# IVRL/NoiseDiff

Measured on AMD Instinct MI355X. Metric: sampled RAW patches/sec (256x256x4, 1000-step DDPM), higher is better.
Workload: dtype f32; 1 GPU; NoiseDiffNet dim=64, 256x256x4 patches, 1000-step DDPM (sigmoid2, pred_v), 16 patches per GPU; a step = one reverse-diffusion step (U-Net forward + fused posterior/noise update) over the per-GPU batch; patches/s = n_gpus*16/(1000*s_per_step); global_batch=16, launch=hipGraph replay, noise=device Philox4x32-10

## Files before the change

include/noisediff_hip.h:

```cpp
#ifndef NOISEDIFF_HIP_H
#define NOISEDIFF_HIP_H

#include <stdint.h>

#ifdef __cplusplus
extern "C" {
#endif

#define ND_E_BADARG   (-1)
#define ND_E_SHAPE    (-2)
#define ND_E_ALIGN    (-3)
#define ND_E_STATE    (-4)

int         nd_version(void);
const char* nd_last_error(void);
int         nd_device_arch(char* buf, int n);


enum nd_prologue {
    ND_PRO_NONE        = 0,
    ND_PRO_AFFINE_SILU = 1,
    ND_PRO_AFFINE_MAP_SILU = 2,
    ND_PRO_LAYERNORM   = 3,
    ND_PRO_SILU        = 4,
    ND_PRO_LEAKY       = 5,
    ND_PRO_LEAKY_SECOND = 6,
    ND_PRO_AFFINE_GENMAP_SILU = 7
};

typedef struct nd_src {
    const float* p0;
    const float* p1;
    int32_t c0, c1;
    int32_t ld0, ld1;
    int32_t mode;
    int32_t upsample;
    int32_t unshuffle;
    int32_t map_blocked;
    const float* mad;
    const float* map;
    const float* vec;
    const float* gamma;
    const float* beta;
    const float* rowstats;
} nd_src;

enum nd_act { ND_ACT_NONE = 0, ND_ACT_GELU = 1, ND_ACT_SILU = 2 };


typedef struct nd_conv3x3 {
    nd_src   src;
    const float* weight;
    const float* bias;
    float*   out;
    float*   stats;
    float*   slot_count;
    int32_t  B, H, W;
    int32_t  cin, cout, ldo;
} nd_conv3x3;

int nd_conv3x3_nhwc_f32(const nd_conv3x3* d, void* stream);
enum nd_conv3x3_kernel { ND_CONV3X3_DIRECT = 0, ND_CONV3X3_WINO = 1, ND_CONV3X3_WINO2 = 2, ND_CONV3X3_WINO4 = 3, ND_CONV3X3_WINO4_16 = 4 };
int nd_conv3x3_takes(int kernel, const nd_conv3x3* d, int splits);
int nd_conv3x3_stat_slots(int H, int W, int cout, int B);
int nd_conv3x3_tiling_id(int B, int H, int W, int cout);
int64_t nd_pack_conv3x3_weight_floats(int cin, int cout);
int nd_pack_conv3x3_weight(const float* oihw, float* packed, int cin, int cout, void* stream);
int nd_pack_conv3x3_weight_dgrad(const float* oihw_fwd, float* packed, int cin, int cout, void* stream);

int nd_conv3x3_wino_nhwc_f32(const nd_conv3x3* d, void* stream);
int nd_conv3x3_wino2_nhwc_f32(const nd_conv3x3* d, void* stream);
int nd_conv3x3_wino_stat_slots(int H, int W);
int64_t nd_pack_conv3x3_wino_weight_floats(int cin, int cout);
int nd_pack_conv3x3_wino_weight(const float* oihw, float* packed, int cin, int cout, void* stream);
int nd_pack_conv3x3_wino_weight_dgrad(const float* oihw_fwd, float* packed, int cin, int cout, void* stream);

int nd_conv3x3_wino4_nhwc_f32(const nd_conv3x3* d, void* stream);
int nd_conv3x3_wino4_16_nhwc_f32(const nd_conv3x3* d, void* stream);
int nd_conv3x3_wino4_stat_slots(int H, int W);
int64_t nd_pack_conv3x3_wino4_weight_floats(int cin, int cout);
int nd_pack_conv3x3_wino4_weight(const float* oihw, float* packed, int cin, int cout, void* stream);
int nd_pack_conv3x3_wino4_weight_dgrad(const float* oihw_fwd, float* packed, int cin, int cout, void* stream);
typedef struct nd_pack_item {
    const float* w;
    float*       packed;
    int32_t      cin, cout, transposed, reserved;
} nd_pack_item;
int nd_pack_conv3x3_wino4_weights_batch(const nd_pack_item* items_dev, int n_items, void* stream);
int nd_conv3x3_wino4_splitk_plan(int B, int H, int W, int cin, int cout);
int64_t nd_conv3x3_wino4_splitk_workspace_floats(int B, int H, int W, int cout, int splits);
int nd_conv3x3_wino4_splitk_nhwc_f32(const nd_conv3x3* d, float* workspace, int splits, void* stream);
int nd_conv3x3_wino4_16_splitk_plan(int H, int W, int cin, int cout);
int nd_conv3x3_wino4_16_splitk_nhwc_f32(const nd_conv3x3* d, float* workspace, int splits, void* stream);


int64_t nd_conv3x3_wgrad_workspace_floats(int B, int H, int W, int cin, int cout);
int nd_conv3x3_wgrad_cat_nhwc_f32(const float* x0, int ldx0, int c0, const float* x1, int ldx1, int c1, const float* dy, int ldy, float* dw_oihw,
                                  float* dbias, float* workspace, int B, int H, int W, int cout, void* stream);
int nd_conv3x3_wgrad_cat_takes(int B, int H, int W, int c0, int c1, int cout, int ldx0, int ldx1, int ldy);
int nd_conv3x3_wgrad_form(int form);
int nd_conv3x3_wgrad_plan(int B, int H, int W, int cin, int cout);
int nd_conv3x3_wgrad_nhwc_f32(const float* x, int ldx, const float* dy, int ldy, float* dw_oihw, float* dbias, float* workspace,
                              int B, int H, int W, int cin, int cout, void* stream);
int nd_conv3x3_wgrad_leaky_nhwc_f32(const float* x, int ldx, const float* dy, int ldy, float* dw_oihw, float* dbias, float* workspace,
                                    int B, int H, int W, int cin, int cout, void* stream);
int64_t nd_conv3x3_wgrad_cat_workspace_floats(int B, int H, int W, int c0, int c1, int cout);
int nd_conv3x3_wgrad_cat_leaky_second_nhwc_f32(const float* x0, int ldx0, int c0, const float* x1, int ldx1, int c1, const float* dy, int ldy,
                                               float* dw_oihw, float* dbias, float* workspace, int B, int H, int W, int cout, void* stream);
int nd_leaky_grad_join_f32(const float* z, float* dz, const float* d_direct, int ld_direct, const float* d_pool, int B, int H, int W, int C,
                           void* stream);

int nd_groupnorm_train_takes(int C, int groups);
int64_t nd_groupnorm_train_workspace_floats(int B, int HW, int C);
int nd_groupnorm_train_forward_f32(const float* x, int ldx, const float* gamma, const float* beta, float* y, int ldy, float* mean_rstd,
                                   float* workspace, int B, int HW, int C, int groups, float eps, void* stream);
int nd_groupnorm_train_backward_f32(const float* dy, int lddy, const float* x, int ldx, const float* gamma, const float* mean_rstd,
                                    float* dx, int lddx, float* dgamma, float* dbeta, float* workspace, int B, int HW, int C, int groups,
                                    void* stream);

int64_t nd_groupnorm_silu_train_workspace_floats(int B, int HW, int C);
int nd_groupnorm_silu_train_forward_f32(const float* x, int ldx, const float* gamma, const float* beta, const float* scale_shift, const float* res, int ldr,
                                        float* y, int ldy, float* mean_rstd, float* mad, float* workspace, int B, int HW, int C, int groups, float eps,
                                        void* stream);
int nd_groupnorm_silu_train_backward_f32(const float* dy, int lddy, const float* x, int ldx, const float* gamma, const float* beta,
                                         const float* scale_shift, const float* mean_rstd, const float* mad, float* dx, int lddx,
                                         float* dgamma, float* dbeta, float* dscale_shift, float* workspace, int B, int HW, int C, int groups,
                                         void* stream);

int nd_modulate_silu_forward_f32(const float* n, int ldn, const float* map, int ldm, float* y, int ldy, int64_t N, int C, void* stream);
int nd_modulate_silu_backward_f32(const float* dy, int lddy, const float* n, int ldn, const float* map, int ldm, float* dn, int lddn, float* dmap, int lddm,
                                  int64_t N, int C, void* stream);

int nd_token_sum_takes(int C);
int64_t nd_token_sum_workspace_floats(int B, int HW, int C);
int nd_token_sum_f32(const float* x, int ldx, float* out, float* workspace, int B, int HW, int C, void* stream);

int nd_layernorm_train_takes(int C);
int64_t nd_layernorm_train_workspace_floats(int64_t N, int C);
int nd_layernorm_train_forward_f32(const float* x, int ldx, const float* gamma, const float* beta, float* y, int ldy, float* stats,
                                   int64_t N, int C, float eps, void* stream);
int nd_layernorm_train_backward_f32(const float* dy, int lddy, const float* x, int ldx, const float* gamma, const float* stats,
                                    float* dx, int lddx, float* dgamma, float* dbeta, float* workspace, int64_t N, int C, void* stream);

int64_t nd_linear_wgrad_workspace_floats(int64_t N, int cin, int cout);
int nd_linear_wgrad_f32(const float* x, int ldx, const float* dy, int ldy, float* dw, float* dbias, float* workspace,
                        int64_t N, int cin, int cout, void* stream);
int nd_linear_wgrad_leaky_f32(const float* x, int ldx, const float* dy, int ldy, float* dw, float* dbias, float* workspace,
                              int64_t N, int cin, int cout, void* stream);
int64_t nd_convt2x2_wgrad_workspace_floats(int B, int h, int w, int cin, int cout);
int nd_convt2x2_wgrad_leaky_f32(const float* x, int ldx, const float* d_up, int ld_up, float* dw, float* workspace, int B, int h, int w,
                                int cin, int cout, int up_h, int up_w, void* stream);


typedef struct nd_pointwise {
    nd_src   src;
    const float* weight;
    const float* bias;
    float*   out;
    const float* res0; const float* res1;
    const float* vec;
    const float* gn_t;
    const float* gn_mad;
    int32_t  B, HW, W;
    int32_t  cin, cout, ldo, ldr0, ldr1, ldt;
    int32_t  act;
    int32_t  shuffle_c;
    int32_t  shuffle_h, shuffle_w;
} nd_pointwise;

int nd_pointwise_gemm_nhwc_f32(const nd_pointwise* d, void* stream);
int nd_pointwise_gemm_unshuffle_crop_nhwc_f32(const nd_pointwise* d, int src_h, int src_w, void* stream);

int64_t nd_image_quality_workspace_bytes(int B, int C, int H, int W);
int nd_image_quality_f32(const float* est, const float* target, const float* scale, double data_range, double* psnr, double* ssim,
                         double* mse, void* workspace, int B, int C, int H, int W, void* stream);
int64_t nd_illum_scale_workspace_bytes(int B, int C, int H, int W);
int nd_illum_scale_f32(const float* pred, const float* source, int source_batch, float* k32, double* k64, void* workspace,
                       int B, int C, int H, int W, void* stream);
int nd_illum_apply_f32(const float* pred, const float* k32, float* out, int B, int C, int H, int W, void* stream);

int     nd_histogram_chunk_elements(void);
int64_t nd_histogram_workspace_bytes(int S, int64_t n, int n_bins);
int nd_histogram_f32(const float* x, int S, int64_t n, const double* edges, int n_edges, int64_t* counts, void* workspace, void* stream);
int nd_kl_div_f64(const int64_t* p_counts, const int64_t* q_counts, int64_t n_p, int64_t n_q, int n_bins, int S, int q_sets, double* out,
                  void* stream);
int nd_kl_div_hist_f64(const double* p, const double* q, int n_bins, int S, int q_sets, double* out, void* stream);
int64_t nd_patch_std_mean_workspace_bytes(int B, int C, int H, int W);
int nd_patch_std_mean_f32(const float* x, float* std, float* mean, double* fit, void* workspace, int B, int C, int H, int W, void* stream);

int64_t nd_level_table_bytes(int n_levels);
int nd_level_moments_reset(uint64_t* table, int n_levels, uint64_t* counters, void* stream);
int nd_level_moments_f32(const float* clean, const float* noisy, int64_t n, float scale, int n_levels, uint64_t* table, uint64_t* counters,
                         void* stream);
int nd_level_stats_f64(const uint64_t* table, int n_levels, int64_t* count, double* mean, double* std, void* stream);
int nd_level_curve_f64(const int64_t* count, const double* std, int n_levels, float scale, int below_median, double* x, double* y, int32_t* m,
                       void* stream);
int64_t nd_theil_sen_workspace_bytes(int max_m, int64_t n_pairs);
int nd_theil_sen_f64(const double* x, const double* y, const int32_t* m, int max_m, const int32_t* pairs, int64_t n_pairs, int max_iter,
                     double tol, double* out, void* workspace, void* stream);

typedef struct nd_denoise_sample {
    int32_t x0, y0;
    int32_t cx, cy;
    int32_t flip;
    int32_t branch;
    float iso, ratio, blc;
    int32_t reserved[3];
} nd_denoise_sample;
#define ND_DENOISE_SNA_WORDS 8
int nd_denoise_batch_f32(const float* noise, const float* clean, const float* ds_k_high, const float* ds_b_high, const float* ds_k_low,
                         const float* ds_b_low, int map_h, int map_w, const nd_denoise_sample* table, const float* sna, const int64_t* rng,
                         uint64_t seed, int64_t first_sample, int32_t draw, const float* counts_in, float* counts_out, float* noisy,
                         float* clean_out, int B, int patch, int crop_h, int crop_w, void* stream);
int nd_philox_poisson_f32(const float* rate, float* out, uint64_t seed, int64_t first_sample, int32_t draw, int B, int64_t n_per_sample,
                          void* stream);
int nd_pack_darkshading_f32(const float* bayer, float* planes, int H2, int W2, void* stream);

typedef struct nd_raw_sample {
    int32_t frame;
    int32_t frame_clean;
    int32_t x0, y0;
    int32_t flip;
    int32_t branch;
    float iso, ratio, blc;
    int32_t reserved;
    double k, sd, ratio64;
} nd_raw_sample;
enum nd_raw_mode {
    ND_RAW_PACK = 0,
    ND_RAW_PACK_SHADED = 1,
    ND_RAW_TRAIN_REAL = 2
};
#define ND_RAW_RESCALE 1
#define ND_RAW_CLIP 2
int nd_raw_pack_u16_f32(const uint16_t* frames, int N, int H2, int W2, const float* ds_k_high, const float* ds_b_high, const float* ds_k_low,
                        const float* ds_b_low, int map_h, int map_w, const nd_raw_sample* table, int mode, int flags, float black, float white,
                        float* out, float* clean_out, int B, int h, int w, void* stream);
int nd_raw_poisson_gaussian_f32(const uint16_t* frames, int N, int H2, int W2, const nd_raw_sample* table, const int64_t* rng, uint64_t seed,
                                int64_t first_sample, int32_t draw, const float* counts_in, const float* normals_in, float* counts_out,
                                float* normals_out, float black, float white, float* noisy, float* clean_out, int B, int h, int w,
                                void* stream);
int nd_raw_to_bayer_u16(const float* img, uint16_t* out, const int32_t* bl, int white, int B, int h, int w, void* stream);
int nd_raw_diffusion_batch_f32(const uint16_t* frames, int N, int H2, int W2, const nd_raw_sample* table, float black, float white, float* noise,
                               float* noisy, float* clean, float* coord, int B, int h, int w, void* stream);
typedef struct nd_develop_params {
    int32_t black[4];
    int32_t white;
    float scale_mul[4];
    float rgb_cam[9];
    int32_t x0, y0;
    int32_t bps;
    int32_t full;
} nd_develop_params;
int nd_raw_develop(const float* src_f32, const uint16_t* src_u16, int B, int H, int W, const nd_develop_params* params, const uint16_t* curve,
                   void* out, int h, int w, void* stream);
int64_t nd_pack_pointwise_weight_floats(int cin, int cout);
int nd_pack_pointwise_weight(const float* w, float* packed, int cin, int cout, int unshuffle_c, void* stream);
int nd_pack_pointwise_weight_t(const float* w_t, float* packed, int cin, int cout, void* stream);
int nd_pack_pointwise_weights_batch(const nd_pack_item* items_dev, int n_items, void* stream);

int nd_pointwise_gemm_split_nhwc_f32(const nd_pointwise* d, void* stream);
int nd_pointwise_gemm_takes(const nd_pointwise* d);
int nd_pointwise_gemm_split_takes(const nd_pointwise* d);
int64_t nd_pack_pointwise_weight_split_floats(int cin, int cout);
int nd_pack_pointwise_weight_split(const float* w, float* packed, int cin, int cout, void* stream);

typedef struct nd_narrow_fold {
    const float* p0; const float* p1;
    const float* t;  const float* mad;
    const float* weight; const float* bias;
    const float* res0;
    float*   out;
    int32_t  B, HW, c0, c1, c2, ld0, ld1, ldt, cout, ldo, ldr0, reserved;
} nd_narrow_fold;
int nd_pointwise_narrow_fold_nhwc_f32(const nd_narrow_fold* d, void* stream);
int nd_pointwise_narrow_fold_takes(int c0, int c1, int c2, int cout);
int64_t nd_pack_narrow_fold_floats(int cin, int cout);
int nd_pack_narrow_fold(const float* wf, const float* bf, const float* wr, const float* br, float* w_out, float* b_out, int cin_r, int mid, int cout,
                        void* stream);

enum nd_chain_res { ND_CHAIN_RES_NONE = 0, ND_CHAIN_RES_INPUT = 1 , ND_CHAIN_RES_INPUT_RAW = 2  };
typedef struct nd_chain_stage {
    const float* weight;
    const float* bias;
    int32_t  cin, cout;
    int32_t  act;
    int32_t  res;
} nd_chain_stage;
typedef struct nd_chain {
    nd_src   src;
    nd_chain_stage st[3];
    float*   out;
    int32_t  n_stages, B, HW, ldo;
} nd_chain;
int nd_pointwise_chain_nhwc_f32(const nd_chain* d, void* stream);
int nd_pointwise_chain_supported(int cin, int n1, int n2, int n3);
int nd_pointwise_chain_takes(int HW, int cin, int n1, int n2, int n3);
int64_t nd_pack_chain_weight_floats(int cin, int cout, int first_stage);
int nd_pack_chain_weight(const float* w, float* packed, int cin, int cout, int first_stage, void* stream);
int nd_pointwise_chain_split_nhwc_f32(const nd_chain* d, void* stream);
int64_t nd_pack_chain_weight_split_floats(int cin, int cout, int first_stage);
int nd_pack_chain_weight_split(const float* w, float* packed, int cin, int cout, int first_stage, void* stream);
typedef struct nd_chain_tail {
    nd_chain chain;
    const float* mad;
    const float* r0;
    const float* r1;
    int32_t  ldr0, ldr1;
} nd_chain_tail;
int nd_pointwise_chain_tail_split_nhwc_f32(const nd_chain_tail* d, void* stream);
int nd_pointwise_chain_tail_takes(int cin, int n1, int n2, int n3);


int nd_groupnorm_finalize_f32(const float* stats, const float* slot_count, int slots,
                              const float* gamma, const float* beta,
                              const float* scale_shift, int ld_ss,
                              float* mad, int B, int C, int groups, float eps, void* stream);
int nd_groupnorm_finalize_train_f32(const float* stats, const float* slot_count, int slots, const float* gamma, const float* beta,
                                    const float* scale_shift, int ld_ss, float* mad, float* mean_rstd, int B, int C, int groups, float eps,
                                    void* stream);

int nd_layernorm_stats_f32(const float* x, int ldx, const float* vec, float* stats,
                           int B, int HW, int C, float eps, void* stream);

int nd_affine_silu_add_f32(const float* t, int ldt, const float* mad,
                           const float* res0, int ldr0, const float* res1, int ldr1,
                           float* out, int ldo, int B, int HW, int C, void* stream);


int nd_linear_rows_f32(const float* in, int ld_in, const float* W, const float* bias,
                       float* out, int ld_out, int B, int K, int N,
                       int act_in, int act_out, void* stream);
int nd_sinusoidal_time_emb_f32(const int64_t* time, const float* freqs, float* emb, int B, int half, void* stream);
int64_t nd_cond_step_lds_bytes(int B, int dim);
int nd_cond_step_f32(const int64_t* time, const float* freqs, const float* W1, const float* b1, const float* W2, const float* b2,
                     const float* Wp, const float* bp, float* out, int ld_out, int B, int dim, int J, void* stream);
int nd_cond_table_build_f32(const float* freqs, const float* W1, const float* b1, const float* W2, const float* b2, float* table, int rows, int dim,
                            void* stream);
int nd_cond_step_table_f32(const int64_t* time, const float* freqs, const float* W1, const float* b1, const float* W2, const float* b2,
                           const float* Wp, const float* bp, float* out, int ld_out, int B, int dim, int J, const float* table, int table_rows,
                           void* stream);
int nd_cond_step_ptable_f32(const int64_t* time, const float* freqs, const float* W1, const float* b1, const float* W2, const float* b2,
                            const float* Wp, const float* bp, float* out, int ld_out, int B, int dim, int J, const float* table, int table_rows,
                            const float* ptable, void* stream);
int nd_embedding_rows_f32(const int64_t* idx, const float* table, float* out, int B, int rows, int dim, void* stream);


int nd_conv7x7_c4_f32(const float* x, const float* wpacked, const float* bias, float* out, int ldo,
                      int B, int H, int W, int cout, void* stream);
int64_t nd_conv7x7_c4_wgrad_workspace_floats(int B, int H, int W, int cout);
int nd_conv7x7_c4_wgrad_f32(const float* x, const float* dy, int ldy, float* dw_oihw, float* dbias, float* workspace, int B, int H, int W, int cout,
                            void* stream);
int nd_pack_conv7x7_weight(const float* oihw, float* packed, int cout, void* stream);
int nd_conv7x7_c4_split_f32(const float* x, const float* wsplit, const float* bias, float* out, int ldo,
                            int B, int H, int W, int cout, void* stream);
int64_t nd_pack_conv7x7_weight_split_floats(int cout);
int nd_pack_conv7x7_weight_split(const float* oihw, float* packed, int cout, void* stream);
int nd_pos_enc_f32(const float* position_nchw, const float* w , const float* bias,
                   float* out, int B, int H, int W, int hid, void* stream);
int nd_maxpool2x2_nhwc_f32(const float* in, float* out, int B, int H, int W, int C, void* stream);
int nd_nchw_to_nhwc_f32(const float* in, float* out, int B, int C, int H, int W, void* stream);
int nd_nhwc_to_nchw_f32(const float* in, float* out, int B, int C, int H, int W, void* stream);
int nd_nchw_to_nhwc_pad_f32(const float* in, float* out, int B, int C, int H, int W, int Cpad, void* stream);


typedef struct nd_sampler_state {
    int32_t* step;
    const int32_t* t_cur;
    const int32_t* t_next;
    const float* coef;
    int64_t* time_out;
    const int64_t* rng;
    int32_t n_steps, B;
} nd_sampler_state;

int nd_sampler_begin_step(const nd_sampler_state* s, void* stream);
int nd_sampler_advance(const nd_sampler_state* s, void* stream);

int nd_sampler_step_ddpm_f32(float* x, const float* model_out, const float* noise, int64_t noise_step_stride,
                             const nd_sampler_state* s, int objective,
                             uint64_t seed, int64_t first_sample,
                             int B, int HW, int C, void* stream);
int nd_sampler_step_ddim_f32(float* x, const float* model_out, const float* noise, int64_t noise_step_stride,
                             const nd_sampler_state* s, int objective,
                             uint64_t seed, int64_t first_sample,
                             int B, int HW, int C, void* stream);
int nd_philox_normal_f32(float* out, uint64_t seed, int64_t first_sample, int32_t step,
                         int B, int HW, int C, void* stream);


int nd_attention_mfma_f32(const float* qkv, int ld_qkv, float* out, int ld_out,
                          int B, int N, int heads, int dh, void* stream);
int64_t nd_linear_attention_workspace_floats(int B, int N, int heads);
int nd_linear_attention_f32(const float* qkv, int ld_qkv, float* out, int ld_out, float* workspace,
                            int B, int N, int heads, int dh, void* stream);
int nd_rmsnorm_nhwc_f32(const float* x, int ldx, const float* g, float* out, int ldo,
                        int B, int HW, int C, void* stream);
int nd_rmsnorm_add_nhwc_f32(const float* x, int ldx, const float* g, const float* res, int ldr, float* out, int ldo, int B, int HW, int C, void* stream);


int nd_attention_train_forward_f32(const float* qkv, int ld_qkv, float* out, int ld_out, float* lse,
                                   int B, int N, int heads, int dh, void* stream);
int64_t nd_attention_backward_workspace_floats(int B, int N, int heads);
int nd_attention_backward_f32(const float* qkv, int ld_qkv, const float* out, int ld_out, const float* dout, int ld_dout, const float* lse,
                              float* dqkv, int ld_dqkv, float* workspace, int B, int N, int heads, int dh, void* stream);
int64_t nd_linear_attention_backward_workspace_floats(int B, int N, int heads);
int nd_linear_attention_backward_f32(const float* qkv, int ld_qkv, const float* dout, int ld_dout, const float* fwd_workspace, float* dqkv,
                                     int ld_dqkv, float* workspace, int B, int N, int heads, int dh, void* stream);
int nd_rmsnorm_train_takes(int C);
int64_t nd_rmsnorm_backward_workspace_floats(int64_t npix, int C);
int nd_rmsnorm_backward_f32(const float* dy, int lddy, const float* x, int ldx, const float* g, float* dx, int lddx, float* dg, float* workspace,
                            int B, int HW, int C, void* stream);

typedef struct nd_adam_item {
    float*       p;
    const float* g;
    float*       m;
    float*       v;
    int64_t      n;
    float        step_size, bias2_sqrt;
    int32_t      vec4, reserved;
    float*       step;
} nd_adam_item;
int nd_adam_chunk_elements(void);
int nd_adam_step_f32(const nd_adam_item* items_dev, int n_items, const int32_t* chunks_dev, int n_chunks, double beta1, double beta2, float eps,
                     float weight_decay, void* stream);
int nd_adam_step_capturable_f32(const nd_adam_item* items_dev, int n_items, const int32_t* chunks_dev, int n_chunks, float lr, double beta1, double beta2,
                                float eps, float weight_decay, void* stream);
int nd_adam_step_capturable_lr_f32(const nd_adam_item* items_dev, int n_items, const int32_t* chunks_dev, int n_chunks, const float* lr_dev, double beta1,
                                   double beta2, float eps, float weight_decay, void* stream);

typedef struct nd_ema_item {
    float*       ema;
    const float* src;
    int64_t      n;
    int32_t      vec4, no_ema;
} nd_ema_item;
int nd_ema_chunk_elements(void);
int nd_ema_update_f32(const nd_ema_item* items_dev, int n_items, const int32_t* chunks_dev, int n_chunks, int64_t* step_dev, uint8_t* initted_dev,
                      void* plan_dev, double beta, int64_t update_after_step, int64_t update_every, double inv_gamma, double power, double min_value,
                      void* stream);

typedef struct nd_diffusion_noising {
    const float* x0;
    const float* noise;
    const float* offset;
    const int64_t* t_in;
    const float* sqrt_alphas_cumprod;
    const float* sqrt_one_minus_alphas_cumprod;
    const int64_t* rng;
    int64_t* t_out;
    float* x_t;
    float* target;
    float* noise_out;
    float* offset_out;
    uint64_t seed;
    int64_t first_sample;
    int64_t draw;
    float offset_strength;
    int32_t B, C, H, W, T;
    int32_t objective, auto_normalize, x0_channels_last;
} nd_diffusion_noising;
int nd_diffusion_noising_f32(const nd_diffusion_noising* p, void* stream);
int nd_diffusion_train_advance(int64_t* rng, void* stream);
int nd_diffusion_loss_slice_elements(void);
int64_t nd_diffusion_loss_workspace_bytes(int B, int C, int HW);
int nd_diffusion_loss_f32(const float* model_out, const float* target, const int64_t* t, const float* loss_weight, int B, int C, int HW, int T,
                          int x0_term, void* workspace, float* loss, float* sample_loss, void* stream);
int nd_diffusion_loss_backward_f32(const float* model_out, const float* target, const int64_t* t, const float* loss_weight, const float* g,
                                   const void* workspace, float* grad_out, int B, int C, int HW, int T, int x0_term, void* stream);

enum nd_layout { ND_LAYOUT_NCHW = 0, ND_LAYOUT_NHWC = 1 };
int nd_denoise_loss_slice_pixels(void);
int64_t nd_denoise_loss_workspace_bytes(int B, int C, int HW);
int nd_denoise_loss_f32(const float* out, int out_layout, const float* target, int B, int C, int HW, double lambda_l1, double lambda_mse,
                        void* workspace, float* terms, float* sample_terms, void* stream);
int nd_denoise_loss_backward_f32(const float* out, int out_layout, const float* target, const float* g, float* grad, int B, int C, int HW,
                                 double lambda_l1, double lambda_mse, void* stream);

int nd_stream_create(void** stream);
int nd_stream_destroy(void* stream);
int nd_stream_sync(void* stream);
int nd_graph_begin(void* stream);
int nd_graph_end(void* stream, void** graph_exec);
int nd_graph_launch(void* graph_exec, void* stream);
int nd_graph_destroy(void* graph_exec);
int nd_stream_device(void* stream);
int nd_event_create(void** ev);
int nd_event_record(void* ev, void* stream);
int nd_event_elapsed_ms(void* start, void* stop, float* ms);
int nd_event_destroy(void* ev);
int nd_event_create_untimed(void** ev);
int nd_stream_wait_event(void* stream, void* ev);

#ifdef __cplusplus
}
#endif
#endif
```

noisediff_amd/_lib.py:

```python
from __future__ import annotations

import ctypes as C
import os
from typing import Optional

HERE = os.path.dirname(os.path.abspath(__file__))
LIB_PATH = os.path.join(HERE, "libnoisediff_hip.so")

PRO_NONE, PRO_AFFINE_SILU, PRO_AFFINE_MAP_SILU, PRO_LAYERNORM, PRO_SILU, PRO_LEAKY, PRO_LEAKY_SECOND, PRO_AFFINE_GENMAP_SILU = 0, 1, 2, 3, 4, 5, 6, 7
ACT_NONE, ACT_GELU, ACT_SILU = 0, 1, 2
OBJECTIVES = {"pred_noise": 0, "pred_x0": 1, "pred_v": 2}
LAYOUT_NCHW, LAYOUT_NHWC = 0, 1
CONV3X3_DIRECT, CONV3X3_WINO, CONV3X3_WINO2, CONV3X3_WINO4, CONV3X3_WINO4_16 = 0, 1, 2, 3, 4

fptr = C.c_void_p


class HipError(RuntimeError):
    pass


class Src(C.Structure):
    _fields_ = [("p0", fptr), ("p1", fptr), ("c0", C.c_int32), ("c1", C.c_int32), ("ld0", C.c_int32), ("ld1", C.c_int32),
                ("mode", C.c_int32), ("upsample", C.c_int32), ("unshuffle", C.c_int32), ("map_blocked", C.c_int32),
                ("mad", fptr), ("map", fptr), ("vec", fptr), ("gamma", fptr), ("beta", fptr), ("rowstats", fptr)]


class AdamItem(C.Structure):
    _fields_ = [("p", fptr), ("g", fptr), ("m", fptr), ("v", fptr), ("n", C.c_int64), ("step_size", C.c_float), ("bias2_sqrt", C.c_float),
                ("vec4", C.c_int32), ("reserved", C.c_int32), ("step", fptr)]


class EmaItem(C.Structure):
    _fields_ = [("ema", fptr), ("src", fptr), ("n", C.c_int64), ("vec4", C.c_int32), ("no_ema", C.c_int32)]


class PackItem(C.Structure):
    _fields_ = [("w", fptr), ("packed", fptr), ("cin", C.c_int32), ("cout", C.c_int32), ("transposed", C.c_int32), ("reserved", C.c_int32)]


class Conv3x3(C.Structure):
    _fields_ = [("src", Src), ("weight", fptr), ("bias", fptr), ("out", fptr), ("stats", fptr), ("slot_count", fptr),
                ("B", C.c_int32), ("H", C.c_int32), ("W", C.c_int32), ("cin", C.c_int32), ("cout", C.c_int32), ("ldo", C.c_int32)]


class Pointwise(C.Structure):
    _fields_ = [("src", Src), ("weight", fptr), ("bias", fptr), ("out", fptr), ("res0", fptr), ("res1", fptr), ("vec", fptr),
                ("gn_t", fptr), ("gn_mad", fptr), ("B", C.c_int32), ("HW", C.c_int32), ("W", C.c_int32), ("cin", C.c_int32),
                ("cout", C.c_int32), ("ldo", C.c_int32), ("ldr0", C.c_int32), ("ldr1", C.c_int32), ("ldt", C.c_int32), ("act", C.c_int32),
                ("shuffle_c", C.c_int32), ("shuffle_h", C.c_int32), ("shuffle_w", C.c_int32)]


class ChainStage(C.Structure):
    _fields_ = [("weight", fptr), ("bias", fptr), ("cin", C.c_int32), ("cout", C.c_int32), ("act", C.c_int32), ("res", C.c_int32)]


class Chain(C.Structure):
    _fields_ = [("src", Src), ("st", ChainStage * 3), ("out", fptr), ("n_stages", C.c_int32), ("B", C.c_int32), ("HW", C.c_int32),
                ("ldo", C.c_int32)]


class ChainTail(C.Structure):
    _fields_ = [("chain", Chain), ("mad", fptr), ("r0", fptr), ("r1", fptr), ("ldr0", C.c_int32), ("ldr1", C.c_int32)]


class NarrowFold(C.Structure):
    _fields_ = [("p0", fptr), ("p1", fptr), ("t", fptr), ("mad", fptr), ("weight", fptr), ("bias", fptr), ("res0", fptr), ("out", fptr),
                ("B", C.c_int32), ("HW", C.c_int32), ("c0", C.c_int32), ("c1", C.c_int32), ("c2", C.c_int32), ("ld0", C.c_int32), ("ld1", C.c_int32),
                ("ldt", C.c_int32), ("cout", C.c_int32), ("ldo", C.c_int32), ("ldr0", C.c_int32), ("reserved", C.c_int32)]


class RawSample(C.Structure):
    _fields_ = [("frame", C.c_int32), ("frame_clean", C.c_int32), ("x0", C.c_int32), ("y0", C.c_int32), ("flip", C.c_int32),
                ("branch", C.c_int32), ("iso", C.c_float), ("ratio", C.c_float), ("blc", C.c_float), ("reserved", C.c_int32),
                ("k", C.c_double), ("sd", C.c_double), ("ratio64", C.c_double)]


class DevelopParams(C.Structure):
    _fields_ = [("black", C.c_int32 * 4), ("white", C.c_int32), ("scale_mul", C.c_float * 4), ("rgb_cam", C.c_float * 9),
                ("x0", C.c_int32), ("y0", C.c_int32), ("bps", C.c_int32), ("full", C.c_int32)]


RAW_PACK, RAW_PACK_SHADED, RAW_TRAIN_REAL = 0, 1, 2
RAW_RESCALE, RAW_CLIP = 1, 2
CHAIN_RES_NONE, CHAIN_RES_INPUT, CHAIN_RES_INPUT_RAW = 0, 1, 2


class SamplerState(C.Structure):
    _fields_ = [("step", fptr), ("t_cur", fptr), ("t_next", fptr), ("coef", fptr), ("time_out", fptr), ("rng", fptr),
                ("n_steps", C.c_int32), ("B", C.c_int32)]


class DiffusionNoising(C.Structure):
    _fields_ = [("x0", fptr), ("noise", fptr), ("offset", fptr), ("t_in", fptr), ("sqrt_alphas_cumprod", fptr), ("sqrt_one_minus_alphas_cumprod", fptr),
                ("rng", fptr), ("t_out", fptr), ("x_t", fptr), ("target", fptr), ("noise_out", fptr), ("offset_out", fptr),
                ("seed", C.c_uint64), ("first_sample", C.c_int64), ("draw", C.c_int64), ("offset_strength", C.c_float),
                ("B", C.c_int32), ("C", C.c_int32), ("H", C.c_int32), ("W", C.c_int32), ("T", C.c_int32),
                ("objective", C.c_int32), ("auto_normalize", C.c_int32), ("x0_channels_last", C.c_int32)]


i32, i64, u64, vp, f32, f64 = C.c_int, C.c_int64, C.c_uint64, C.c_void_p, C.c_float, C.c_double

SIGNATURES = {
    "nd_version": (i32, []),
    "nd_last_error": (C.c_char_p, []),
    "nd_device_arch": (i32, [C.c_char_p, i32]),
    "nd_conv3x3_nhwc_f32": (i32, [C.POINTER(Conv3x3), vp]),
    "nd_conv3x3_takes": (i32, [i32, C.POINTER(Conv3x3), i32]),
    "nd_conv3x3_stat_slots": (i32, [i32, i32, i32, i32]),
    "nd_conv3x3_tiling_id": (i32, [i32, i32, i32, i32]),
    "nd_pack_conv3x3_weight_floats": (i64, [i32, i32]),
    "nd_pack_conv3x3_weight": (i32, [vp, vp, i32, i32, vp]),
    "nd_pack_conv3x3_weight_dgrad": (i32, [vp, vp, i32, i32, vp]),
    "nd_conv3x3_wino_nhwc_f32": (i32, [C.POINTER(Conv3x3), vp]),
    "nd_conv3x3_wino2_nhwc_f32": (i32, [C.POINTER(Conv3x3), vp]),
    "nd_conv3x3_wino_stat_slots": (i32, [i32, i32]),
    "nd_conv3x3_wino4_stat_slots": (i32, [i32, i32]),
    "nd_pack_conv3x3_wino_weight_floats": (i64, [i32, i32]),
    "nd_pack_conv3x3_wino_weight": (i32, [vp, vp, i32, i32, vp]),
    "nd_pack_conv3x3_wino_weight_dgrad": (i32, [vp, vp, i32, i32, vp]),
    "nd_conv3x3_wino4_nhwc_f32": (i32, [C.POINTER(Conv3x3), vp]),
    "nd_conv3x3_wino4_16_nhwc_f32": (i32, [C.POINTER(Conv3x3), vp]),
    "nd_pack_conv3x3_wino4_weight_floats": (i64, [i32, i32]),
    "nd_pack_conv3x3_wino4_weight": (i32, [vp, vp, i32, i32, vp]),
    "nd_pack_conv3x3_wino4_weight_dgrad": (i32, [vp, vp, i32, i32, vp]),
    "nd_conv3x3_wino4_splitk_plan": (i32, [i32, i32, i32, i32, i32]),
    "nd_conv3x3_wino4_splitk_workspace_floats": (i64, [i32, i32, i32, i32, i32]),
    "nd_conv3x3_wino4_splitk_nhwc_f32": (i32, [vp, vp, i32, vp]),
    "nd_conv3x3_wino4_16_splitk_plan": (i32, [i32, i32, i32, i32]),
    "nd_conv3x3_wino4_16_splitk_nhwc_f32": (i32, [vp, vp, i32, vp]),
    "nd_conv3x3_wgrad_workspace_floats": (i64, [i32, i32, i32, i32, i32]),
    "nd_conv3x3_wgrad_nhwc_f32": (i32, [vp, i32, vp, i32, vp, vp, vp, i32, i32, i32, i32, i32, vp]),
    "nd_groupnorm_train_workspace_floats": (i64, [i32, i32, i32]),
    "nd_linear_wgrad_workspace_floats": (i64, [i64, i32, i32]),
    "nd_groupnorm_silu_train_workspace_floats": (i64, [i32, i32, i32]),
    "nd_groupnorm_silu_train_forward_f32": (i32, [vp, i32, vp, vp, vp, vp, i32, vp, i32, vp, vp, vp, i32, i32, i32, i32, C.c_float, vp]),
    "nd_token_sum_workspace_floats": (i64, [i32, i32, i32]),
    "nd_token_sum_f32": (i32, [vp, i32, vp, vp, i32, i32, i32, vp]),
    "nd_modulate_silu_forward_f32": (i32, [vp, i32, vp, i32, vp, i32, i64, i32, vp]),
    "nd_modulate_silu_backward_f32": (i32, [vp, i32, vp, i32, vp, i32, vp, i32, vp, i32, i64, i32, vp]),
    "nd_groupnorm_silu_train_backward_f32": (i32, [vp, i32, vp, i32, vp, vp, vp, vp, vp, vp, i32, vp, vp, vp, vp, i32, i32, i32, i32, vp]),
    "nd_layernorm_train_workspace_floats": (i64, [i64, i32]),
    "nd_layernorm_train_forward_f32": (i32, [vp, i32, vp, vp, vp, i32, vp, i64, i32, C.c_float, vp]),
    "nd_layernorm_train_backward_f32": (i32, [vp, i32, vp, i32, vp, vp, vp, i32, vp, vp, vp, i64, i32, vp]),
    "nd_linear_wgrad_f32": (i32, [vp, i32, vp, i32, vp, vp, vp, i64, i32, i32, vp]),
    "nd_groupnorm_train_forward_f32": (i32, [vp, i32, vp, vp, vp, i32, vp, vp, i32, i32, i32, i32, C.c_float, vp]),
    "nd_groupnorm_train_backward_f32": (i32, [vp, i32, vp, i32, vp, vp, vp, i32, vp, vp, vp, i32, i32, i32, i32, vp]),
    "nd_pointwise_gemm_nhwc_f32": (i32, [C.POINTER(Pointwise), vp]),
    "nd_pointwise_chain_nhwc_f32": (i32, [C.POINTER(Chain), vp]),
    "nd_pointwise_chain_supported": (i32, [i32, i32, i32, i32]),
    "nd_pack_chain_weight_floats": (i64, [i32, i32, i32]),
    "nd_pack_chain_weight": (i32, [vp, vp, i32, i32, i32, vp]),
    "nd_pointwise_chain_split_nhwc_f32": (i32, [C.POINTER(Chain), vp]),
    "nd_pack_chain_weight_split_floats": (i64, [i32, i32, i32]),
    "nd_pack_chain_weight_split": (i32, [vp, vp, i32, i32, i32, vp]),
    "nd_pointwise_gemm_split_nhwc_f32": (i32, [C.POINTER(Pointwise), vp]),
    "nd_pointwise_gemm_split_takes": (i32, [C.POINTER(Pointwise)]),
    "nd_pointwise_gemm_takes": (i32, [C.POINTER(Pointwise)]),
    "nd_pointwise_chain_takes": (i32, [i32, i32, i32, i32, i32]),
    "nd_groupnorm_train_takes": (i32, [i32, i32]),
    "nd_layernorm_train_takes": (i32, [i32]),
    "nd_rmsnorm_train_takes": (i32, [i32]),
    "nd_token_sum_takes": (i32, [i32]),
    "nd_conv3x3_wgrad_plan": (i32, [i32, i32, i32, i32, i32]),
    "nd_conv3x3_wgrad_cat_takes": (i32, [i32, i32, i32, i32, i32, i32, i32, i32, i32]),
    "nd_pack_pointwise_weight_split_floats": (i64, [i32, i32]),
    "nd_pack_pointwise_weight_split": (i32, [vp, vp, i32, i32, vp]),
    "nd_pointwise_chain_tail_split_nhwc_f32": (i32, [C.POINTER(ChainTail), vp]),
    "nd_pointwise_chain_tail_takes": (i32, [i32, i32, i32, i32]),
    "nd_pointwise_narrow_fold_nhwc_f32": (i32, [C.POINTER(NarrowFold), vp]),
    "nd_pointwise_narrow_fold_takes": (i32, [i32, i32, i32, i32]),
    "nd_pack_narrow_fold_floats": (i64, [i32, i32]),
    "nd_pack_narrow_fold": (i32, [vp, vp, vp, vp, vp, vp, i32, i32, i32, vp]),
    "nd_pack_pointwise_weight_floats": (i64, [i32, i32]),
    "nd_pack_pointwise_weight": (i32, [vp, vp, i32, i32, i32, vp]),
    "nd_pack_pointwise_weight_t": (i32, [vp, vp, i32, i32, vp]),
    "nd_pack_pointwise_weights_batch": (i32, [vp, i32, vp]),
    "nd_pack_conv3x3_wino4_weights_batch": (i32, [vp, i32, vp]),
    "nd_conv3x3_wgrad_cat_nhwc_f32": (i32, [vp, i32, i32, vp, i32, i32, vp, i32, vp, vp, vp, i32, i32, i32, i32, vp]),
    "nd_conv3x3_wgrad_form": (i32, [i32]),
    "nd_conv7x7_c4_wgrad_workspace_floats": (i64, [i32, i32, i32, i32]),
    "nd_conv7x7_c4_wgrad_f32": (i32, [vp, vp, i32, vp, vp, vp, i32, i32, i32, i32, vp]),
    "nd_adam_chunk_elements": (i32, []),
    "nd_adam_step_f32": (i32, [vp, i32, vp, i32, f64, f64, f32, f32, vp]),
    "nd_adam_step_capturable_f32": (i32, [vp, i32, vp, i32, f32, f64, f64, f32, f32, vp]),
    "nd_adam_step_capturable_lr_f32": (i32, [vp, i32, vp, i32, vp, f64, f64, f32, f32, vp]),
    "nd_ema_chunk_elements": (i32, []),
    "nd_ema_update_f32": (i32, [vp, i32, vp, i32, vp, vp, vp, f64, i64, i64, f64, f64, f64, vp]),
    "nd_diffusion_noising_f32": (i32, [C.POINTER(DiffusionNoising), vp]),
    "nd_diffusion_train_advance": (i32, [vp, vp]),
    "nd_diffusion_loss_slice_elements": (i32, []),
    "nd_diffusion_loss_workspace_bytes": (i64, [i32, i32, i32]),
    "nd_diffusion_loss_f32": (i32, [vp, vp, vp, vp, i32, i32, i32, i32, i32, vp, vp, vp, vp]),
    "nd_diffusion_loss_backward_f32": (i32, [vp, vp, vp, vp, vp, vp, vp, i32, i32, i32, i32, i32, vp]),
    "nd_denoise_loss_slice_pixels": (i32, []),
    "nd_denoise_loss_workspace_bytes": (i64, [i32, i32, i32]),
    "nd_denoise_loss_f32": (i32, [vp, i32, vp, i32, i32, i32, f64, f64, vp, vp, vp, vp]),
    "nd_denoise_loss_backward_f32": (i32, [vp, i32, vp, vp, vp, i32, i32, i32, f64, f64, vp]),
    "nd_groupnorm_finalize_f32": (i32, [vp, vp, i32, vp, vp, vp, i32, vp, i32, i32, i32, f32, vp]),
    "nd_groupnorm_finalize_train_f32": (i32, [vp, vp, i32, vp, vp, vp, i32, vp, vp, i32, i32, i32, f32, vp]),
    "nd_layernorm_stats_f32": (i32, [vp, i32, vp, vp, i32, i32, i32, f32, vp]),
    "nd_affine_silu_add_f32": (i32, [vp, i32, vp, vp, i32, vp, i32, vp, i32, i32, i32, i32, vp]),
    "nd_linear_rows_f32": (i32, [vp, i32, vp, vp, vp, i32, i32, i32, i32, i32, i32, vp]),
    "nd_sinusoidal_time_emb_f32": (i32, [vp, vp, vp, i32, i32, vp]),
    "nd_cond_step_lds_bytes": (i64, [i32, i32]),
    "nd_cond_step_f32": (i32, [vp, vp, vp, vp, vp, vp, vp, vp, vp, i32, i32, i32, i32, vp]),
    "nd_cond_table_build_f32": (i32, [vp, vp, vp, vp, vp, vp, i32, i32, vp]),
    "nd_cond_step_table_f32": (i32, [vp, vp, vp, vp, vp, vp, vp, vp, vp, i32, i32, i32, i32, vp, i32, vp]),
    "nd_cond_step_ptable_f32": (i32, [vp, vp, vp, vp, vp, vp, vp, vp, vp, i32, i32, i32, i32, vp, i32, vp, vp]),
    "nd_embedding_rows_f32": (i32, [vp, vp, vp, i32, i32, i32, vp]),
    "nd_conv7x7_c4_f32": (i32, [vp, vp, vp, vp, i32, i32, i32, i32, i32, vp]),
    "nd_pack_conv7x7_weight": (i32, [vp, vp, i32, vp]),
    "nd_conv7x7_c4_split_f32": (i32, [vp, vp, vp, vp, i32, i32, i32, i32, i32, vp]),
    "nd_pack_conv7x7_weight_split_floats": (i64, [i32]),
    "nd_pack_conv7x7_weight_split": (i32, [vp, vp, i32, vp]),
    "nd_pos_enc_f32": (i32, [vp, vp, vp, vp, i32, i32, i32, i32, vp]),
    "nd_maxpool2x2_nhwc_f32": (i32, [vp, vp, i32, i32, i32, i32, vp]),
    "nd_nchw_to_nhwc_pad_f32": (i32, [vp, vp, i32, i32, i32, i32, i32, vp]),
    "nd_nchw_to_nhwc_f32": (i32, [vp, vp, i32, i32, i32, i32, vp]),
    "nd_nhwc_to_nchw_f32": (i32, [vp, vp, i32, i32, i32, i32, vp]),
    "nd_sampler_begin_step": (i32, [C.POINTER(SamplerState), vp]),
    "nd_sampler_advance": (i32, [C.POINTER(SamplerState), vp]),
    "nd_sampler_step_ddpm_f32": (i32, [vp, vp, vp, i64, C.POINTER(SamplerState), i32, u64, i64, i32, i32, i32, vp]),
    "nd_sampler_step_ddim_f32": (i32, [vp, vp, vp, i64, C.POINTER(SamplerState), i32, u64, i64, i32, i32, i32, vp]),
    "nd_philox_normal_f32": (i32, [vp, u64, i64, i32, i32, i32, i32, vp]),
    "nd_attention_mfma_f32": (i32, [vp, i32, vp, i32, i32, i32, i32, i32, vp]),
    "nd_attention_train_forward_f32": (i32, [vp, i32, vp, i32, vp, i32, i32, i32, i32, vp]),
    "nd_attention_backward_workspace_floats": (i64, [i32, i32, i32]),
    "nd_attention_backward_f32": (i32, [vp, i32, vp, i32, vp, i32, vp, vp, i32, vp, i32, i32, i32, i32, vp]),
    "nd_linear_attention_backward_workspace_floats": (i64, [i32, i32, i32]),
    "nd_linear_attention_backward_f32": (i32, [vp, i32, vp, i32, vp, vp, i32, vp, i32, i32, i32, i32, vp]),
    "nd_rmsnorm_backward_workspace_floats": (i64, [i64, i32]),
    "nd_rmsnorm_backward_f32": (i32, [vp, i32, vp, i32, vp, vp, i32, vp, vp, i32, i32, i32, vp]),
    "nd_linear_attention_workspace_floats": (i64, [i32, i32, i32]),
    "nd_linear_attention_f32": (i32, [vp, i32, vp, i32, vp, i32, i32, i32, i32, vp]),
    "nd_rmsnorm_nhwc_f32": (i32, [vp, i32, vp, vp, i32, i32, i32, i32, vp]),
    "nd_rmsnorm_add_nhwc_f32": (i32, [vp, i32, vp, vp, i32, vp, i32, i32, i32, i32, vp]),
    "nd_stream_create": (i32, [C.POINTER(vp)]),
    "nd_stream_destroy": (i32, [vp]),
    "nd_stream_sync": (i32, [vp]),
    "nd_graph_begin": (i32, [vp]),
    "nd_graph_end": (i32, [vp, C.POINTER(vp)]),
    "nd_graph_launch": (i32, [vp, vp]),
    "nd_graph_destroy": (i32, [vp]),
    "nd_event_create": (i32, [C.POINTER(vp)]),
    "nd_event_record": (i32, [vp, vp]),
    "nd_event_elapsed_ms": (i32, [vp, vp, C.POINTER(f32)]),
    "nd_event_destroy": (i32, [vp]),
    "nd_event_create_untimed": (i32, [C.POINTER(vp)]),
    "nd_stream_wait_event": (i32, [vp, vp]),
    "nd_stream_device": (i32, [vp]),
    "nd_conv3x3_wgrad_leaky_nhwc_f32": (i32, [vp, i32, vp, i32, vp, vp, vp, i32, i32, i32, i32, i32, vp]),
    "nd_conv3x3_wgrad_cat_workspace_floats": (i64, [i32, i32, i32, i32, i32, i32]),
    "nd_conv3x3_wgrad_cat_leaky_second_nhwc_f32": (i32, [vp, i32, i32, vp, i32, i32, vp, i32, vp, vp, vp, i32, i32, i32, i32, vp]),
    "nd_leaky_grad_join_f32": (i32, [vp, vp, vp, i32, vp, i32, i32, i32, i32, vp]),
    "nd_linear_wgrad_leaky_f32": (i32, [vp, i32, vp, i32, vp, vp, vp, i64, i32, i32, vp]),
    "nd_convt2x2_wgrad_workspace_floats": (i64, [i32, i32, i32, i32, i32]),
    "nd_convt2x2_wgrad_leaky_f32": (i32, [vp, i32, vp, i32, vp, vp, i32, i32, i32, i32, i32, i32, i32, vp]),
    "nd_pointwise_gemm_unshuffle_crop_nhwc_f32": (i32, [C.POINTER(Pointwise), i32, i32, vp]),
    "nd_image_quality_workspace_bytes": (i64, [i32, i32, i32, i32]),
    "nd_image_quality_f32": (i32, [vp, vp, vp, f64, vp, vp, vp, vp, i32, i32, i32, i32, vp]),
    "nd_illum_scale_workspace_bytes": (i64, [i32, i32, i32, i32]),
    "nd_illum_scale_f32": (i32, [vp, vp, i32, vp, vp, vp, i32, i32, i32, i32, vp]),
    "nd_illum_apply_f32": (i32, [vp, vp, vp, i32, i32, i32, i32, vp]),
    "nd_histogram_chunk_elements": (i32, []),
    "nd_histogram_workspace_bytes": (i64, [i32, i64, i32]),
    "nd_histogram_f32": (i32, [vp, i32, i64, vp, i32, vp, vp, vp]),
    "nd_kl_div_f64": (i32, [vp, vp, i64, i64, i32, i32, i32, vp, vp]),
    "nd_kl_div_hist_f64": (i32, [vp, vp, i32, i32, i32, vp, vp]),
    "nd_patch_std_mean_workspace_bytes": (i64, [i32, i32, i32, i32]),
    "nd_patch_std_mean_f32": (i32, [vp, vp, vp, vp, vp, i32, i32, i32, i32, vp]),
    "nd_level_table_bytes": (i64, [i32]),
    "nd_level_moments_reset": (i32, [vp, i32, vp, vp]),
    "nd_level_moments_f32": (i32, [vp, vp, i64, f32, i32, vp, vp, vp]),
    "nd_level_stats_f64": (i32, [vp, i32, vp, vp, vp, vp]),
    "nd_level_curve_f64": (i32, [vp, vp, i32, f32, i32, vp, vp, vp, vp]),
    "nd_theil_sen_workspace_bytes": (i64, [i32, i64]),
    "nd_theil_sen_f64": (i32, [vp, vp, vp, i32, vp, i64, i32, f64, vp, vp, vp]),
    "nd_denoise_batch_f32": (i32, [vp, vp, vp, vp, vp, vp, i32, i32, vp, vp, vp, u64, i64, i32, vp, vp, vp, vp, i32, i32, i32, i32, vp]),
    "nd_philox_poisson_f32": (i32, [vp, vp, u64, i64, i32, i32, i64, vp]),
    "nd_pack_darkshading_f32": (i32, [vp, vp, i32, i32, vp]),
    "nd_raw_pack_u16_f32": (i32, [vp, i32, i32, i32, vp, vp, vp, vp, i32, i32, vp, i32, i32, f32, f32, vp, vp, i32, i32, i32, vp]),
    "nd_raw_poisson_gaussian_f32": (i32, [vp, i32, i32, i32, vp, vp, u64, i64, i32, vp, vp, vp, vp, f32, f32, vp, vp, i32, i32, i32, vp]),
    "nd_raw_to_bayer_u16": (i32, [vp, vp, C.POINTER(C.c_int32), i32, i32, i32, i32, vp]),
    "nd_raw_diffusion_batch_f32": (i32, [vp, i32, i32, i32, vp, f32, f32, vp, vp, vp, vp, i32, i32, i32, vp]),
    "nd_raw_develop": (i32, [vp, vp, i32, i32, i32, C.POINTER(DevelopParams), vp, vp, i32, i32, vp]),
}

_UNCHECKED = {"nd_conv3x3_takes", "nd_pointwise_gemm_takes", "nd_pointwise_gemm_split_takes", "nd_pointwise_chain_supported", "nd_pointwise_chain_takes",
              "nd_groupnorm_train_takes", "nd_layernorm_train_takes", "nd_rmsnorm_train_takes", "nd_token_sum_takes", "nd_conv3x3_wgrad_plan", "nd_conv3x3_wgrad_cat_takes",
              "nd_pointwise_chain_tail_takes", "nd_pointwise_narrow_fold_takes", "nd_pack_narrow_fold_floats", "nd_version", "nd_last_error", "nd_stream_device", "nd_conv3x3_wgrad_form", "nd_adam_chunk_elements", "nd_ema_chunk_elements", "nd_conv7x7_c4_wgrad_workspace_floats", "nd_conv3x3_stat_slots", "nd_conv3x3_tiling_id", "nd_pack_conv3x3_weight_floats",
              "nd_pack_pointwise_weight_floats", "nd_linear_attention_workspace_floats", "nd_conv3x3_wino_stat_slots", "nd_conv3x3_wino4_stat_slots",
              "nd_pack_conv3x3_wino_weight_floats", "nd_pack_conv3x3_wino4_weight_floats", "nd_conv3x3_wino4_splitk_plan", "nd_conv3x3_wino4_16_splitk_plan", "nd_conv3x3_wino4_splitk_workspace_floats", "nd_token_sum_workspace_floats", "nd_cond_step_lds_bytes", "nd_conv3x3_wgrad_workspace_floats",
              "nd_groupnorm_train_workspace_floats", "nd_linear_wgrad_workspace_floats",
              "nd_layernorm_train_workspace_floats", "nd_groupnorm_silu_train_workspace_floats", "nd_conv3x3_wgrad_cat_workspace_floats",
              "nd_convt2x2_wgrad_workspace_floats", "nd_image_quality_workspace_bytes", "nd_illum_scale_workspace_bytes",
              "nd_histogram_chunk_elements", "nd_histogram_workspace_bytes", "nd_patch_std_mean_workspace_bytes", "nd_level_table_bytes",
              "nd_theil_sen_workspace_bytes", "nd_attention_backward_workspace_floats", "nd_linear_attention_backward_workspace_floats",
              "nd_rmsnorm_backward_workspace_floats", "nd_diffusion_loss_slice_elements", "nd_diffusion_loss_workspace_bytes",
              "nd_denoise_loss_slice_pixels", "nd_denoise_loss_workspace_bytes"}

_lib: Optional[C.CDLL] = None


def load(path: str = LIB_PATH) -> C.CDLL:
    global _lib
    if _lib is not None:
        return _lib
    import torch
    if not os.path.exists(path):
        raise HipError(f"{path} is missing: the HIP library is the product and there is no fallback. "
                       "Build it with `python -m noisediff_amd.build`.")
    lib = C.CDLL(path)
    for name, (res, args) in SIGNATURES.items():
        fn = getattr(lib, name)
        fn.restype, fn.argtypes = res, args
    _lib = lib
    return lib


def check(code: int, what: str = "") -> None:
    if code != 0:
        msg = load().nd_last_error().decode(errors="replace")
        raise HipError(f"{what or 'libnoisediff_hip'} failed with code {code}: {msg}")


def call(name: str, *args):
    r = getattr(load(), name)(*args)
    if name not in _UNCHECKED:
        check(r, name)
    return r


def ptr(t) -> Optional[int]:
    return None if t is None else t.data_ptr()
```

noisediff_amd/csrc/pwchain.hip:

```cpp
#include <type_traits>
#include "nd_common.h"
#include "split_bf16.h"

namespace {

struct ChainArgs {
    nd_chain d;
    int n_tiles;
    int tiles_per_sample;
    const float* mad;
    const float* r0;
    const float* r1;
    int ldr0, ldr1;
};

template <int K, int N>
__device__ __forceinline__ void chain_gemm(const float (&in)[K / 2], const float* __restrict__ w, const float* __restrict__ bias,
                                           f32x16 (&acc)[N / 32], const int lane) {
    const int half = lane >> 5;
#pragma unroll
    for (int nt = 0; nt < N / 32; ++nt)
#pragma unroll
        for (int g = 0; g < 4; ++g) {
            const f32x4 b4 = nd_ld4(bias + 32 * nt + 8 * g + 4 * half);
#pragma unroll
            for (int i = 0; i < 4; ++i) acc[nt][4 * g + i] = b4[i];
        }
#pragma unroll
    for (int jq = 0; jq < K / 8; ++jq)
#pragma unroll
        for (int nt = 0; nt < N / 32; ++nt) {
            const f32x4 a4 = nd_ld4(w + ((nt * (K / 8) + jq) * 64 + lane) * 4);
#pragma unroll
            for (int i = 0; i < 4; ++i) acc[nt] = nd_mfma(a4[i], in[4 * jq + i], acc[nt]);
        }
}

template <int K, int N>
__device__ __forceinline__ void chain_gemm_split(const float (&in)[K / 2], const char* __restrict__ w, const float* __restrict__ bias,
                                                 f32x16 (&acc)[N / 32], const int lane) {
    static_assert(K % 16 == 0, "whole 16-channel K steps");
    constexpr int S = K / 16, NT = N / 32;
    const int half = lane >> 5;
    const u32x4* const wl = reinterpret_cast<const u32x4*>(w) + lane;
    u32x4 wq[2][3], xs[2][3];
    auto load_w = [&](int slot, int s_, int nt_) {
        const u32x4* p = wl + ((nt_ * S + s_) * 3) * 64;
        wq[slot][0] = p[0];  wq[slot][1] = p[64];  wq[slot][2] = p[128];
    };
    auto split = [&](int slot, int s_) {
#pragma unroll
        for (int j = 0; j < 4; ++j) {
            unsigned t1, t2, t3;
            nd_split2_bf16(in[8 * s_ + 2 * j], in[8 * s_ + 2 * j + 1], t1, t2, t3);
            xs[slot][0][j] = t1;  xs[slot][1][j] = t2;  xs[slot][2][j] = t3;
        }
    };
    load_w(0, 0, 0);
#pragma unroll
    for (int nt = 0; nt < NT; ++nt)
#pragma unroll
        for (int g = 0; g < 4; ++g) {
            const f32x4 b4 = nd_ld4(bias + 32 * nt + 8 * g + 4 * half);
#pragma unroll
            for (int i = 0; i < 4; ++i) acc[nt][4 * g + i] = b4[i];
        }
    split(0, 0);
#pragma unroll
    for (int s = 0; s < S; ++s)
#pragma unroll
        for (int nt = 0; nt < NT; ++nt) {
            const int g = s * NT + nt;
            if (g + 1 < S * NT) load_w((g + 1) & 1, nt + 1 < NT ? s : s + 1, nt + 1 < NT ? nt + 1 : 0);
            __builtin_amdgcn_sched_barrier(0);
            if (nt == 0 && s + 1 < S) split((s + 1) & 1, s + 1);
            const u32x4 w1 = wq[g & 1][0], w2 = wq[g & 1][1], w3 = wq[g & 1][2];
            const u32x4 x1 = xs[s & 1][0], x2 = xs[s & 1][1], x3 = xs[s & 1][2];
            acc[nt] = nd_mfma_bf16(w1, x1, acc[nt]);
            acc[nt] = nd_mfma_bf16(w1, x2, acc[nt]);
            acc[nt] = nd_mfma_bf16(w2, x1, acc[nt]);
            acc[nt] = nd_mfma_bf16(w2, x2, acc[nt]);
            acc[nt] = nd_mfma_bf16(w1, x3, acc[nt]);
            acc[nt] = nd_mfma_bf16(w3, x1, acc[nt]);
            __builtin_amdgcn_sched_barrier(0);
        }
}

template <int N>
__device__ __forceinline__ void chain_act(f32x16 (&acc)[N / 32], const int act) {
    if (act == ND_ACT_NONE) return;
#pragma unroll
    for (int nt = 0; nt < N / 32; ++nt)
#pragma unroll
        for (int r = 0; r < 16; r += 2) {
            if (act == ND_ACT_GELU) {
                const f32x2 g = nd_gelu2(f32x2{acc[nt][r], acc[nt][r + 1]});
                acc[nt][r] = g.x;  acc[nt][r + 1] = g.y;
            } else { acc[nt][r] = nd_silu(acc[nt][r]);  acc[nt][r + 1] = nd_silu(acc[nt][r + 1]); }
        }
}

template <int K0, int N>
__device__ __forceinline__ void chain_res(f32x16 (&acc)[N / 32], const f32x4 (&x)[K0 / 8], const float* vstash, const int res, const int half) {
    if (res == ND_CHAIN_RES_NONE) return;
#pragma unroll
    for (int nt = 0; nt < N / 32; ++nt)
#pragma unroll
        for (int g = 0; g < 4; ++g) {
            const int q = 4 * nt + g;
            if (q < K0 / 8) {
                f32x4 v = x[q];
                if (res == ND_CHAIN_RES_INPUT_RAW && vstash) v -= nd_ld4(vstash + 8 * q + 4 * half);
#pragma unroll
                for (int i = 0; i < 4; ++i) acc[nt][4 * g + i] += v[i];
            }
        }
}

template <int N>
__device__ __forceinline__ void chain_store_buf(const f32x16 (&acc)[N / 32], __amdgpu_buffer_rsrc_t rso, const unsigned row_bytes, const int cout, const int half) {
#pragma unroll
    for (int nt = 0; nt < N / 32; ++nt)
#pragma unroll
        for (int g = 0; g < 4; ++g) {
            const int n0 = 32 * nt + 8 * g + 4 * half;
            const f32x4 v = {acc[nt][4 * g], acc[nt][4 * g + 1], acc[nt][4 * g + 2], acc[nt][4 * g + 3]};
            __builtin_amdgcn_raw_buffer_store_b128(__builtin_bit_cast(u32x4, v), rso, n0 < cout ? row_bytes + n0 * 4u : 0xFFFFFFF0u, 0, 0);
        }
}

template <int N>
__device__ __forceinline__ void chain_store(const f32x16 (&acc)[N / 32], float* row, const int cout, const int half) {
#pragma unroll
    for (int nt = 0; nt < N / 32; ++nt)
#pragma unroll
        for (int g = 0; g < 4; ++g) {
            const int n0 = 32 * nt + 8 * g + 4 * half;
            if (n0 < cout) {
                const f32x4 v = {acc[nt][4 * g], acc[nt][4 * g + 1], acc[nt][4 * g + 2], acc[nt][4 * g + 3]};
                nd_st4(row + n0, v);
            }
        }
}

constexpr int chain_threads(int n1, bool split = false, int k0 = 0) { return split ? (n1 >= 128 || k0 >= 48 ? 512 : 768) : (n1 >= 128 ? 768 : 1024); }

#ifdef CHAIN_STAMP
__device__ unsigned long long chain_dbg[4096 * 16 * 10];
#define CH_T0() (stamp_t = __builtin_amdgcn_s_memtime())
#define CH_ACC(i) { const unsigned long long now_ = __builtin_amdgcn_s_memtime(); stamp[i] += now_ - stamp_t; stamp_t = now_; }
#else
#define CH_T0()
#define CH_ACC(i)
#endif

template <bool SPLIT> constexpr int chain_w_floats(int n, int k) { return SPLIT ? n * k * 3 / 2 : n * k; }

template <int K0, int N1, int N2, int N3, int MODE, bool SPLIT = false, bool TAIL = false>
__global__ __launch_bounds__(chain_threads(N1, SPLIT, K0), 1) void chain_kernel(const ChainArgs a) {
    constexpr int THREADS = chain_threads(N1, SPLIT, K0), WAVES = THREADS / 64;
    static_assert(!SPLIT || K0 % 16 == 0, "SPLIT: the first stage reads whole 16-channel K steps");
    static_assert(!TAIL || (SPLIT && MODE == ND_PRO_NONE), "TAIL: a prologue of the SPLIT form");
    extern __shared__ __attribute__((aligned(16))) float lds[];
    float* w1 = lds;
    float* w2 = w1 + chain_w_floats<SPLIT>(N1, K0);
    float* w3 = w2 + chain_w_floats<SPLIT>(N2, N1);
    float* b1 = w3 + chain_w_floats<SPLIT>(N3, N2);
    float* b2 = b1 + N1;
    float* b3 = b2 + N2;
    float* gam = b3 + (N3 > 0 ? N3 : 0);
    float* bet = gam + K0;
    float* vst = bet + K0;
    float* mst = vst + WAVES * K0;

    const int tid = threadIdx.x, lane = tid & 63, wave = tid >> 6, half = lane >> 5;
    const nd_src& s = a.d.src;
    const int cin = s.c0 + s.c1;

    {
        auto copy4 = [&](float* dst, const float* src, int n) {
            for (int i = tid * 4; i < n; i += THREADS * 4) nd_st4(dst + i, nd_ld4(src + i));
        };
        auto copy_pad = [&](float* dst, const float* src, int n, int npad, float fill) {
            for (int i = tid; i < npad; i += THREADS) dst[i] = (src && i < n) ? src[i] : fill;
        };
        copy4(w1, a.d.st[0].weight, chain_w_floats<SPLIT>(N1, K0));
        copy4(w2, a.d.st[1].weight, chain_w_floats<SPLIT>(N2, N1));
        copy_pad(b1, a.d.st[0].bias, a.d.st[0].cout, N1, 0.0f);
        copy_pad(b2, a.d.st[1].bias, a.d.st[1].cout, N2, 0.0f);
        if (N3 > 0) {
            copy4(w3, a.d.st[2].weight, chain_w_floats<SPLIT>(N3, N2));
            copy_pad(b3, a.d.st[2].bias, a.d.st[2].cout, N3, 0.0f);
        }
        if (MODE == ND_PRO_LAYERNORM) {
            copy_pad(gam, s.gamma, cin, K0, 0.0f);
            copy_pad(bet, s.beta, cin, K0, 0.0f);
        }
    }
    __syncthreads();

    const int n_waves = gridDim.x * WAVES, wid = blockIdx.x * WAVES + wave;
    const int t_begin = (int)((long)wid * a.n_tiles / n_waves), t_end = (int)((long)(wid + 1) * a.n_tiles / n_waves);
    float* myv = vst + wave * K0;
    float* mym = mst + wave * 3 * K0;
    int b_cur = -1;
    const int cout_last = a.d.st[N3 > 0 ? 2 : 1].cout;

    constexpr bool TWO = SPLIT && K0 == 16;
    constexpr unsigned OOB = 0xFFFFFFF0u;
    const __amdgpu_buffer_rsrc_t rs0 = __builtin_amdgcn_make_buffer_rsrc(const_cast<float*>(s.p0), 0, (int)((unsigned)a.d.B * a.d.HW * s.ld0 * 4u), 0x00020000);
    const __amdgpu_buffer_rsrc_t rs1 = __builtin_amdgcn_make_buffer_rsrc(const_cast<float*>(s.p1 ? s.p1 : s.p0), 0,
                                                                          s.p1 ? (int)((unsigned)a.d.B * a.d.HW * s.ld1 * 4u) : 0, 0x00020000);
    const __amdgpu_buffer_rsrc_t rso = __builtin_amdgcn_make_buffer_rsrc(a.d.out, 0, (int)((unsigned)a.d.B * a.d.HW * a.d.ldo * 4u), 0x00020000);
    const __amdgpu_buffer_rsrc_t rr0 = __builtin_amdgcn_make_buffer_rsrc(const_cast<float*>(TAIL ? a.r0 : s.p0), 0,
                                                                          TAIL ? (int)((unsigned)a.d.B * a.d.HW * a.ldr0 * 4u) : 0, 0x00020000);
    const __amdgpu_buffer_rsrc_t rr1 = __builtin_amdgcn_make_buffer_rsrc(const_cast<float*>(TAIL && a.r1 ? a.r1 : s.p0), 0,
                                                                          TAIL && a.r1 ? (int)((unsigned)a.d.B * a.d.HW * a.ldr1 * 4u) : 0, 0x00020000);
    f32x4 Xn[SPLIT ? K0 / 8 : 1], Xm[TWO ? K0 / 8 : 1];
    f32x4 R0n[TAIL ? K0 / 8 : 1], R1n[TAIL ? K0 / 8 : 1];
    auto prefetch_rows = [&](int t_) {
        const unsigned pix_ = (unsigned)t_ * 32u + (unsigned)(lane & 31);
#pragma unroll
        for (int q = 0; q < K0 / 8; ++q) {
            const int c = 8 * q + 4 * half;
            Xn[SPLIT ? q : 0] = __builtin_bit_cast(f32x4, __builtin_amdgcn_raw_buffer_load_b128(rs0, c < s.c0 ? (pix_ * (unsigned)s.ld0 + c) * 4u : OOB, 0, 0));
            if constexpr (TWO)
                Xm[q] = __builtin_bit_cast(f32x4, __builtin_amdgcn_raw_buffer_load_b128(rs1, (c >= s.c0 && c < cin) ? (pix_ * (unsigned)s.ld1 + (c - s.c0)) * 4u : OOB, 0, 0));
            if constexpr (TAIL) {
                R0n[q] = __builtin_bit_cast(f32x4, __builtin_amdgcn_raw_buffer_load_b128(rr0, c < cin ? (pix_ * (unsigned)a.ldr0 + c) * 4u : OOB, 0, 0));
                R1n[q] = __builtin_bit_cast(f32x4, __builtin_amdgcn_raw_buffer_load_b128(rr1, c < cin ? (pix_ * (unsigned)a.ldr1 + c) * 4u : OOB, 0, 0));
            }
        }
    };
    if constexpr (SPLIT) {
        if (t_begin < t_end) prefetch_rows(t_begin);
    }

#ifdef CHAIN_STAMP
    unsigned long long stamp[8] = {0, 0, 0, 0, 0, 0, 0, 0}, stamp_t = 0;
    const unsigned long long stamp_c0 = __builtin_amdgcn_s_memtime(), stamp_r0 = __builtin_amdgcn_s_memrealtime();
#endif
    for (int t = t_begin; t < t_end; ++t) {
        CH_T0();
        const int b = t / a.tiles_per_sample;
        const size_t pix = (size_t)t * 32 + (lane & 31);
        if (s.vec && b != b_cur) {
            for (int c = lane; c < K0; c += 64) myv[c] = c < cin ? s.vec[(size_t)b * cin + c] : 0.0f;
            b_cur = b;
        }
        if (TAIL && b != b_cur) {
            for (int c = lane; c < 3 * K0; c += 64) {
                const int j = c / K0, cc = c - j * K0;
                mym[c] = cc < cin ? a.mad[((size_t)b * 3 + j) * cin + cc] : 0.0f;
            }
            b_cur = b;
        }
        f32x4 X[K0 / 8];
        if constexpr (SPLIT) {
#pragma unroll
            for (int q = 0; q < K0 / 8; ++q) {
                X[q] = Xn[q];
                if constexpr (TWO) X[q] += Xm[q];
                if constexpr (TAIL) {
                    const float* m = mym + 8 * q + 4 * half;
                    X[q] = nd_silu4((X[q] - nd_ld4(m)) * nd_ld4(m + K0) + nd_ld4(m + 2 * K0)) + R0n[q] + R1n[q];
                }
            }
            prefetch_rows(t + 1 < t_end ? t + 1 : t);
            if (s.vec) {
#pragma unroll
                for (int q = 0; q < K0 / 8; ++q) X[q] += nd_ld4(myv + 8 * q + 4 * half);
            }
        } else {
#pragma unroll
            for (int q = 0; q < K0 / 8; ++q) {
                const int c = 8 * q + 4 * half;
                const f32x4 zero = {0, 0, 0, 0};
                X[q] = zero;
                if (c < s.c0) X[q] = nd_ld4(s.p0 + pix * s.ld0 + c);
                else if (c < cin) X[q] = nd_ld4(s.p1 + pix * s.ld1 + (c - s.c0));
                if (s.vec) X[q] += nd_ld4(myv + c);
            }
        }
        float in0[K0 / 2];
        if (MODE == ND_PRO_LAYERNORM) {
            float sum = 0.0f;
#pragma unroll
            for (int q = 0; q < K0 / 8; ++q) sum += (X[q][0] + X[q][1]) + (X[q][2] + X[q][3]);
            sum += __shfl_xor(sum, 32);
            const float mean = sum / (float)cin;
            float m2 = 0.0f;
#pragma unroll
            for (int q = 0; q < K0 / 8; ++q) {
                if (8 * q + 4 * half < cin) {
#pragma unroll
                    for (int i = 0; i < 4; ++i) { const float dv = X[q][i] - mean; m2 = fmaf(dv, dv, m2); }
                }
            }
            m2 += __shfl_xor(m2, 32);
            const float rstd = rsqrtf(m2 / (float)cin + 1e-5f);
#pragma unroll
            for (int q = 0; q < K0 / 8; ++q) {
                const f32x4 g4 = nd_ld4(gam + 8 * q + 4 * half), be4 = nd_ld4(bet + 8 * q + 4 * half);
#pragma unroll
                for (int i = 0; i < 4; ++i) in0[4 * q + i] = (X[q][i] - mean) * rstd * g4[i] + be4[i];
            }
        } else {
#pragma unroll
            for (int q = 0; q < K0 / 8; ++q)
#pragma unroll
                for (int i = 0; i < 4; ++i) in0[4 * q + i] = X[q][i];
        }

        CH_ACC(0);
        f32x16 H1[N1 / 32];
        if constexpr (SPLIT) chain_gemm_split<K0, N1>(in0, reinterpret_cast<const char*>(w1), b1, H1, lane);
        else chain_gemm<K0, N1>(in0, w1, b1, H1, lane);
        CH_ACC(1);
        chain_res<K0, N1>(H1, X, s.vec ? myv : nullptr, a.d.st[0].res, half);
        chain_act<N1>(H1, a.d.st[0].act);
        CH_ACC(2);
        float in1[N1 / 2];
#pragma unroll
        for (int nt = 0; nt < N1 / 32; ++nt)
#pragma unroll
            for (int r = 0; r < 16; ++r) in1[16 * nt + r] = H1[nt][r];
        f32x16 H2[N2 / 32];
        if constexpr (SPLIT) chain_gemm_split<N1, N2>(in1, reinterpret_cast<const char*>(w2), b2, H2, lane);
        else chain_gemm<N1, N2>(in1, w2, b2, H2, lane);
        CH_ACC(3);
        chain_res<K0, N2>(H2, X, s.vec ? myv : nullptr, a.d.st[1].res, half);
        chain_act<N2>(H2, a.d.st[1].act);
        CH_ACC(4);
        float* row = a.d.out + pix * a.d.ldo;
        if (N3 > 0) {
            float in2[N2 / 2];
#pragma unroll
            for (int nt = 0; nt < N2 / 32; ++nt)
#pragma unroll
                for (int r = 0; r < 16; ++r) in2[16 * nt + r] = H2[nt][r];
            f32x16 H3[(N3 > 0 ? N3 : 32) / 32];
            if constexpr (SPLIT) chain_gemm_split<N2, (N3 > 0 ? N3 : 32)>(in2, reinterpret_cast<const char*>(w3), b3, H3, lane);
            else chain_gemm<N2, (N3 > 0 ? N3 : 32)>(in2, w3, b3, H3, lane);
            CH_ACC(5);
            chain_res<K0, (N3 > 0 ? N3 : 32)>(H3, X, s.vec ? myv : nullptr, a.d.st[2].res, half);
            chain_act<(N3 > 0 ? N3 : 32)>(H3, a.d.st[2].act);
            if constexpr (SPLIT) chain_store_buf<(N3 > 0 ? N3 : 32)>(H3, rso, (unsigned)pix * (unsigned)a.d.ldo * 4u, cout_last, half);
            else chain_store<(N3 > 0 ? N3 : 32)>(H3, row, cout_last, half);
        } else {
            if constexpr (SPLIT) chain_store_buf<N2>(H2, rso, (unsigned)pix * (unsigned)a.d.ldo * 4u, cout_last, half);
            else chain_store<N2>(H2, row, cout_last, half);
        }
        CH_ACC(6);
    }
#ifdef CHAIN_STAMP
    if (lane == 0 && wid < 4096 * 16) {
        unsigned long long* o = chain_dbg + (size_t)wid * 10;
        for (int i = 0; i < 7; ++i) o[i] = stamp[i];
        o[7] = __builtin_amdgcn_s_memtime() - stamp_c0;
        o[8] = __builtin_amdgcn_s_memrealtime() - stamp_r0;
        o[9] = (unsigned long long)(t_end - t_begin);
    }
#endif
}

__global__ void pack_chain_kernel(const float* __restrict__ w, float* __restrict__ out, int cin, int cout, int KP, int NP) {
    const int total = KP * NP;
    for (int idx = blockIdx.x * blockDim.x + threadIdx.x; idx < total; idx += gridDim.x * blockDim.x) {
        const int i = idx & 3, l = (idx >> 2) & 63, rest = idx >> 8;
        const int jq = rest % (KP / 8), nt = rest / (KP / 8);
        const int n = 32 * nt + (l & 31), k = 8 * jq + i + 4 * (l >> 5);
        out[idx] = (n < cout && k < cin) ? w[(size_t)n * cin + k] : 0.0f;
    }
}

__global__ void pack_chain_split_kernel(const float* __restrict__ w, unsigned short* __restrict__ out, int cin, int cout, int KP, int NP) {
    const int total = KP * NP;
    for (int idx = blockIdx.x * blockDim.x + threadIdx.x; idx < total; idx += gridDim.x * blockDim.x) {
        const int i = idx & 7, l = (idx >> 3) & 63, rest = idx >> 9;
        const int s = rest % (KP / 16), nt = rest / (KP / 16);
        const int n = 32 * nt + (l & 31), k = 16 * s + 8 * (i >> 2) + 4 * (l >> 5) + (i & 3);
        const float v = (n < cout && k < cin) ? w[(size_t)n * cin + k] : 0.0f;
        const bf16_terms t = nd_split3_bf16(v);
        unsigned short* o = out + ((size_t)(nt * (KP / 16) + s) * 3 * 64 + l) * 8 + i;
        o[0] = t.t1;  o[512] = t.t2;  o[1024] = t.t3;
    }
}

template <int K0, int N1, int N2, int N3, int MODE, bool SPLIT = false, bool TAIL = false>
int launch(const ChainArgs& a, hipStream_t st) {
    static nd_device_once configured;
    constexpr int THREADS = chain_threads(N1, SPLIT, K0), WAVES = THREADS / 64;
    constexpr int STASH = (TAIL ? 4 : 1) * K0;
    const size_t lds = (size_t)(chain_w_floats<SPLIT>(N1, K0) + chain_w_floats<SPLIT>(N2, N1) + chain_w_floats<SPLIT>(N3, N2) + N1 + N2 + N3 + 2 * K0 + WAVES * STASH) * sizeof(float);
    static_assert((size_t)(chain_w_floats<SPLIT>(N1, K0) + chain_w_floats<SPLIT>(N2, N1) + chain_w_floats<SPLIT>(N3, N2) + N1 + N2 + N3 + 2 * K0 + 16 * STASH) * 4 <= 160 * 1024, "LDS");
    if (int e = nd_reserve_lds(configured, reinterpret_cast<const void*>(chain_kernel<K0, N1, N2, N3, MODE, SPLIT, TAIL>), lds, "nd_pointwise_chain")) return e;
    const int wgs = nd_cdiv(a.n_tiles, WAVES);
    const int grid = wgs < nd_device_cus() ? wgs : nd_device_cus();
    hipLaunchKernelGGL((chain_kernel<K0, N1, N2, N3, MODE, SPLIT, TAIL>), dim3(grid), dim3(THREADS), lds, st, a);
    return 0;
}

template <int K0, int N1, int N2, int N3, bool SPLIT = false>
int launch_mode(const ChainArgs& a, hipStream_t st) {
    if (a.d.src.mode == ND_PRO_LAYERNORM) return launch<K0, N1, N2, N3, ND_PRO_LAYERNORM, SPLIT>(a, st);
    return launch<K0, N1, N2, N3, ND_PRO_NONE, SPLIT>(a, st);
}

}

extern "C" int64_t nd_pack_chain_weight_floats(int cin, int cout, int first_stage) {
    return (int64_t)nd_round_up(cin, first_stage ? 8 : 32) * nd_round_up(cout, 32);
}

extern "C" int nd_pack_chain_weight(const float* w, float* packed, int cin, int cout, int first_stage, void* stream) {
    ND_REQUIRE(w && packed, ND_E_BADARG, "nd_pack_chain_weight: null pointer");
    ND_REQUIRE(cin > 0 && cout > 0, ND_E_SHAPE, "nd_pack_chain_weight: non-positive size");
    const int KP = nd_round_up(cin, first_stage ? 8 : 32), NP = nd_round_up(cout, 32);
    const int total = KP * NP;
    hipLaunchKernelGGL(pack_chain_kernel, dim3(nd_cdiv(total, 256) < 1024 ? nd_cdiv(total, 256) : 1024), dim3(256), 0, (hipStream_t)stream,
                       w, packed, cin, cout, KP, NP);
    return nd_launch_status("nd_pack_chain_weight");
}

#define ND_CHAIN_ROWS(X) \
    X(8, 32, 32, 0)  X(16, 32, 32, 0) X(16, 32, 32, 32) X(32, 32, 32, 0) X(32, 32, 32, 32) X(32, 64, 32, 32) X(8, 64, 64, 0) \
    X(48, 64, 64, 0) X(48, 96, 64, 64) X(64, 64, 64, 0) X(64, 64, 32, 0) X(48, 64, 32, 0)  X(64, 128, 64, 64)

constexpr int chain_k0(int k0, bool split) { return split ? (k0 + 15) / 16 * 16 : k0; }

template <bool SPLIT>
static int chain_row(int cin, int n1, int n2, int n3, const ChainArgs* a, hipStream_t st) {
    const int K0 = nd_round_up(cin, SPLIT ? 16 : 8), N1 = nd_round_up(n1, 32), N2 = nd_round_up(n2, 32), N3 = n3 > 0 ? nd_round_up(n3, 32) : 0;
#define ND_CHAIN_ROW(k0, r1, r2, r3) \
    if (K0 == chain_k0(k0, SPLIT) && N1 == r1 && N2 == r2 && N3 == r3) return a ? launch_mode<chain_k0(k0, SPLIT), r1, r2, r3, SPLIT>(*a, st) : 0;
    ND_CHAIN_ROWS(ND_CHAIN_ROW)
#undef ND_CHAIN_ROW
    return ND_E_SHAPE;
}

static inline bool chain_pixels_ok(int HW) { return HW > 0 && HW % 32 == 0; }

extern "C" int nd_pointwise_chain_supported(int cin, int n1, int n2, int n3) { return chain_row<false>(cin, n1, n2, n3, nullptr, nullptr) == 0; }

extern "C" int nd_pointwise_chain_takes(int HW, int cin, int n1, int n2, int n3) { return chain_pixels_ok(HW) && nd_pointwise_chain_supported(cin, n1, n2, n3); }

extern "C" int64_t nd_pack_chain_weight_split_floats(int cin, int cout, int first_stage) {
    return (int64_t)nd_round_up(cin, first_stage ? 16 : 32) * nd_round_up(cout, 32) * 3 / 2;
}

extern "C" int nd_pack_chain_weight_split(const float* w, float* packed, int cin, int cout, int first_stage, void* stream) {
    ND_REQUIRE(w && packed && nd_aligned16(packed), ND_E_BADARG, "nd_pack_chain_weight_split: null or unaligned pointer");
    ND_REQUIRE(cin > 0 && cout > 0, ND_E_SHAPE, "nd_pack_chain_weight_split: non-positive size");
    const int KP = nd_round_up(cin, first_stage ? 16 : 32), NP = nd_round_up(cout, 32);
    const int total = KP * NP;
    hipLaunchKernelGGL(pack_chain_split_kernel, dim3(nd_cdiv(total, 256) < 1024 ? nd_cdiv(total, 256) : 1024), dim3(256), 0, (hipStream_t)stream,
                       w, reinterpret_cast<unsigned short*>(packed), cin, cout, KP, NP);
    return nd_launch_status("nd_pack_chain_weight_split");
}

static int chain_run(const nd_chain* d, void* stream, bool split) {
    ND_REQUIRE(d, ND_E_BADARG, "nd_pointwise_chain: null descriptor");
    const nd_src& s = d->src;
    ND_REQUIRE(d->n_stages == 2 || d->n_stages == 3, ND_E_BADARG, "nd_pointwise_chain: n_stages=%d (2 or 3)", d->n_stages);
    ND_REQUIRE(s.p0 && d->out, ND_E_BADARG, "nd_pointwise_chain: null tensor pointer");
    ND_REQUIRE(d->B > 0 && chain_pixels_ok(d->HW), ND_E_SHAPE, "nd_pointwise_chain: HW=%d must be a positive multiple of 32", d->HW);
    ND_REQUIRE(s.c0 > 0 && s.c0 % 4 == 0 && s.c1 % 4 == 0 && (s.c1 == 0) == (s.p1 == nullptr), ND_E_SHAPE,
               "nd_pointwise_chain: source channels %d+%d (multiples of 4; p1 iff c1)", s.c0, s.c1);
    const int cin = s.c0 + s.c1;
    ND_REQUIRE(s.ld0 >= s.c0 && s.ld0 % 4 == 0 && (s.c1 == 0 || (s.ld1 >= s.c1 && s.ld1 % 4 == 0)), ND_E_ALIGN,
               "nd_pointwise_chain: pixel strides must be >= channels and multiples of 4");
    ND_REQUIRE(s.mode == ND_PRO_NONE || s.mode == ND_PRO_LAYERNORM, ND_E_BADARG, "nd_pointwise_chain: unsupported prologue %d", s.mode);
    ND_REQUIRE(s.mode != ND_PRO_LAYERNORM || (s.gamma && s.beta), ND_E_BADARG, "nd_pointwise_chain: LayerNorm needs gamma and beta");
    ND_REQUIRE(!s.upsample && !s.unshuffle && !s.rowstats, ND_E_BADARG, "nd_pointwise_chain: plain pixel addressing only");
    int width = cin;
    for (int i = 0; i < d->n_stages; ++i) {
        const nd_chain_stage& g = d->st[i];
        ND_REQUIRE(g.weight && g.cin == width && g.cout > 0, ND_E_SHAPE, "nd_pointwise_chain: stage %d is %d->%d, expected input width %d", i,
                   g.cin, g.cout, width);
        ND_REQUIRE(g.res == ND_CHAIN_RES_NONE || g.cout == cin, ND_E_SHAPE, "nd_pointwise_chain: stage %d residual needs cout == input width", i);
        ND_REQUIRE(nd_aligned16(g.weight), ND_E_ALIGN, "nd_pointwise_chain: weights must be 16-byte aligned");
        width = g.cout;
    }
    ND_REQUIRE(width % 4 == 0 && d->ldo >= width && d->ldo % 4 == 0, ND_E_SHAPE, "nd_pointwise_chain: output width %d, ldo %d", width, d->ldo);
    ND_REQUIRE(nd_aligned16(s.p0) && nd_aligned16(s.p1) && nd_aligned16(d->out), ND_E_ALIGN, "nd_pointwise_chain: tensors must be 16-byte aligned");
    const int n3 = d->n_stages == 3 ? d->st[2].cout : 0;
    ND_REQUIRE(nd_pointwise_chain_supported(cin, d->st[0].cout, d->st[1].cout, n3), ND_E_SHAPE,
               "nd_pointwise_chain: widths %d->%d->%d->%d are not instantiated (use nd_pointwise_gemm_nhwc_f32 per layer)", cin,
               d->st[0].cout, d->st[1].cout, n3);
    ChainArgs a{};
    a.d = *d;
    a.tiles_per_sample = d->HW / 32;
    const long tiles = (long)d->B * a.tiles_per_sample;
    ND_REQUIRE(tiles < (1L << 31), ND_E_SHAPE, "nd_pointwise_chain: too many pixels");
    a.n_tiles = (int)tiles;
    hipStream_t st = (hipStream_t)stream;
    const int n1 = d->st[0].cout, n2 = d->st[1].cout;
    if (split) {
        ND_REQUIRE(s.c1 == 0 || cin <= 16, ND_E_SHAPE, "nd_pointwise_chain_split: two sources only with cin <= 16 (got %d + %d)", s.c0, s.c1);
        ND_REQUIRE((long)d->B * d->HW * s.ld0 * 4 < (1L << 32) - 65536 && (long)d->B * d->HW * (s.c1 ? s.ld1 : 0) * 4 < (1L << 32) - 65536 &&
                   (long)d->B * d->HW * d->ldo * 4 < (1L << 32) - 65536, ND_E_SHAPE, "nd_pointwise_chain_split: a tensor of 4 GiB or more");
        if (int rc = chain_row<true>(cin, n1, n2, n3, &a, st)) return rc;
        return nd_launch_status("nd_pointwise_chain_split_nhwc_f32");
    }
    if (int rc = chain_row<false>(cin, n1, n2, n3, &a, st)) return rc;
    return nd_launch_status("nd_pointwise_chain_nhwc_f32");
}

extern "C" int nd_pointwise_chain_tail_takes(int cin, int n1, int n2, int n3) {
    return n3 == 0 && (cin == 64 || cin == 48) && nd_round_up(n1, 32) == 64 && n1 > 0 && nd_round_up(n2, 32) == 32 && n2 > 0;
}

extern "C" int nd_pointwise_chain_tail_split_nhwc_f32(const nd_chain_tail* dt, void* stream) {
    ND_REQUIRE(dt, ND_E_BADARG, "nd_pointwise_chain_tail: null descriptor");
    const nd_chain* d = &dt->chain;
    const nd_src& s = d->src;
    ND_REQUIRE(d->n_stages == 2 && s.p0 && d->out && dt->mad && dt->r0, ND_E_BADARG, "nd_pointwise_chain_tail: two stages, t, mad, r0 and out");
    ND_REQUIRE(d->B > 0 && chain_pixels_ok(d->HW), ND_E_SHAPE, "nd_pointwise_chain_tail: HW=%d must be a positive multiple of 32", d->HW);
    ND_REQUIRE(s.c1 == 0 && !s.p1 && s.mode == ND_PRO_NONE && !s.vec && !s.upsample && !s.unshuffle && !s.rowstats, ND_E_BADARG,
               "nd_pointwise_chain_tail: one plain source (the affine + SiLU is this entry point's own prologue)");
    const int cin = s.c0;
    ND_REQUIRE(nd_pointwise_chain_tail_takes(cin, d->st[0].cout, d->st[1].cout, 0), ND_E_SHAPE,
               "nd_pointwise_chain_tail: widths %d->%d->%d are not instantiated (nd_affine_silu_add_f32, then the chain)", cin, d->st[0].cout, d->st[1].cout);
    ND_REQUIRE(s.ld0 >= cin && s.ld0 % 4 == 0 && dt->ldr0 >= cin && dt->ldr0 % 4 == 0 && (!dt->r1 || (dt->ldr1 >= cin && dt->ldr1 % 4 == 0)), ND_E_ALIGN,
               "nd_pointwise_chain_tail: pixel strides must be >= channels and multiples of 4");
    int width = cin;
    for (int i = 0; i < 2; ++i) {
        const nd_chain_stage& g = d->st[i];
        ND_REQUIRE(g.weight && g.cin == width && g.cout > 0 && g.res == ND_CHAIN_RES_NONE, ND_E_SHAPE, "nd_pointwise_chain_tail: stage %d is %d->%d, expected input width %d, no residual",
                   i, g.cin, g.cout, width);
        ND_REQUIRE(nd_aligned16(g.weight), ND_E_ALIGN, "nd_pointwise_chain_tail: weights must be 16-byte aligned");
        width = g.cout;
    }
    ND_REQUIRE(width % 4 == 0 && d->ldo >= width && d->ldo % 4 == 0, ND_E_SHAPE, "nd_pointwise_chain_tail: output width %d, ldo %d", width, d->ldo);
    ND_REQUIRE(nd_aligned16(s.p0) && nd_aligned16(d->out) && nd_aligned16(dt->mad) && nd_aligned16(dt->r0) && nd_aligned16(dt->r1), ND_E_ALIGN,
               "nd_pointwise_chain_tail: tensors must be 16-byte aligned");
    const long px = (long)d->B * d->HW, lim = (1L << 32) - 65536;
    ND_REQUIRE(px * s.ld0 * 4 < lim && px * dt->ldr0 * 4 < lim && px * (dt->r1 ? dt->ldr1 : 0) * 4 < lim && px * d->ldo * 4 < lim, ND_E_SHAPE,
               "nd_pointwise_chain_tail: a tensor of 4 GiB or more");
    ChainArgs a{};
    a.d = *d;
    a.tiles_per_sample = d->HW / 32;
    ND_REQUIRE(px / 32 < (1L << 31), ND_E_SHAPE, "nd_pointwise_chain_tail: too many pixels");
    a.n_tiles = (int)(px / 32);
    a.mad = dt->mad;  a.r0 = dt->r0;  a.r1 = dt->r1;  a.ldr0 = dt->ldr0;  a.ldr1 = dt->r1 ? dt->ldr1 : 0;
    const int rc = cin == 64 ? launch<64, 64, 32, 0, ND_PRO_NONE, true, true>(a, (hipStream_t)stream) : launch<48, 64, 32, 0, ND_PRO_NONE, true, true>(a, (hipStream_t)stream);
    if (rc) return rc;
    return nd_launch_status("nd_pointwise_chain_tail_split_nhwc_f32");
}

#ifdef CHAIN_STAMP
extern "C" int nd_chain_debug_read(unsigned long long* host, int n_words) {
    return (int)hipMemcpyFromSymbol(host, HIP_SYMBOL(chain_dbg), (size_t)n_words * 8);
}
#endif

extern "C" int nd_pointwise_chain_nhwc_f32(const nd_chain* d, void* stream) { return chain_run(d, stream, false); }

extern "C" int nd_pointwise_chain_split_nhwc_f32(const nd_chain* d, void* stream) { return chain_run(d, stream, true); }
```

noisediff_amd/engine.py:

```python
from __future__ import annotations

import ctypes as C
import logging
import math
import os
import threading
from dataclasses import dataclass
from typing import Callable, Dict, List, Optional, Sequence, Tuple

import torch

from . import _lib as L
from ._host import chain_takes, conv3x3_takes, pointwise_takes
from .spec import (normalize_stage_attn, stage_attention_param_spec, ATTN_DIM_HEAD, ATTN_HEADS, ISO_DIM, ISO_TABLE_ROWS, POS_DIM, POS_GROUPS, RESNET_GROUPS, SHOT_GROUPS,
                   arch_param_spec, arch_traits, attention_param_spec, stage_dims)

GN_EPS = 1e-5
_log = logging.getLogger("noisediff_amd")
WINOGRAD = os.environ.get("ND_WINOGRAD", "1") != "0"
PREACT = True
PREACT_MIN = 256
CHAIN = True
_CHAIN_FIRST = (".ff.net.0.0.weight", ".fc1.weight")
_CHAIN_LATER = (".ff.net.2.weight", ".proj_out.weight", ".fc2.weight")
WINO2 = os.environ.get("ND_WINO2", "1") != "0"
MAP_BLOCKED = True
GENMAP = os.environ.get("ND_GENMAP", "1") != "0"
COND_STEP = True
WINO4 = os.environ.get("ND_WINO4", "1") != "0"
SPLIT_K = os.environ.get("ND_SPLIT_K", "0") != "0"
EIGHT_TILES_RULE = True
WINO4_16 = os.environ.get("ND_WINO4_16", "narrow")
WINO4_16_SPLIT = True
_ALIGN = 64
_SPLIT = os.environ.get("ND_SPLIT_GEMM", "1")
SPLIT_GEMM = _SPLIT != "0"
SPLIT_CHAIN, SPLIT_PW = _SPLIT in ("1", "chain"), _SPLIT in ("1", "pw")
FOLD_FINAL = os.environ.get("ND_FOLD_FINAL", "1") != "0"
SHOT_TAIL = os.environ.get("ND_SHOT_TAIL", "1") != "0"
TIME_TABLE = True
PROJ_TABLE = True
TIME_TABLE_ROWS = 1000


def _few_items(H: int, W: int, cout: int) -> bool:
    return ((H + 15) // 16) * ((W + 31) // 32) * ((cout + 63) // 64) <= 8


def _wino4_layer(cin: int, cout: int) -> bool:
    return conv3x3_takes(L.CONV3X3_WINO4, 1, 32, 32, cin, cout, cin, 0, cin, 0)


def conv3x3_form(B: int, H: int, W: int, cin: int, cout: int, c0: int, c1: int, ld0: int, ld1: int, mode: int, upsample: bool, packed4: bool, *,
                 winograd=None, wino2=None, wino4=None, split_k=None, eight_tiles=None, wino4_16=None, wino4_16_split=None):
    knob = lambda value, default: default if value is None else value
    k_winograd, k_wino2, k_wino4, k_split, k_eight = knob(winograd, WINOGRAD), knob(wino2, WINO2), knob(wino4, WINO4), knob(split_k, SPLIT_K), knob(eight_tiles, EIGHT_TILES_RULE)
    k_16, k_16split = knob(wino4_16, WINO4_16), knob(wino4_16_split, WINO4_16_SPLIT)
    if not (k_winograd and H >= 16 and W >= 16):
        return "", 1, B

    def piece(kernel: int, splits: int = 1, mode: int = mode) -> int:
        takes = lambda b: b * H * W * cout * 4 < _LAUNCH_OUT_BYTES and conv3x3_takes(kernel, b, H, W, cin, cout, c0, c1, ld0, ld1, mode, upsample, splits=splits)
        if takes(B):
            return B
        if not takes(1):
            return 0
        lo, hi = 1, B
        while lo < hi:
            mid = (lo + hi + 1) // 2
            lo, hi = (mid, hi) if takes(mid) else (lo, mid - 1)
        return -(-B // -(-B // lo))

    few = _few_items(H, W, cout)
    stored = L.PRO_AFFINE_MAP_SILU if mode == L.PRO_AFFINE_GENMAP_SILU else mode
    form, rows = "", 0
    if k_wino4 and packed4 and mode in (L.PRO_NONE, L.PRO_AFFINE_SILU, L.PRO_AFFINE_MAP_SILU, L.PRO_AFFINE_GENMAP_SILU):
        if k_16 != "0" and (W % 16 == 0 or W >= 48) and (k_16 == "all" or W < 32 or (few and k_eight and not k_split)):
            form, rows = "wino4_16", piece(L.CONV3X3_WINO4_16)
        to_wino2 = not rows and k_wino2 and not k_split and k_eight and few and piece(L.CONV3X3_WINO2, mode=stored) > 0
        if not rows and not to_wino2 and W >= 32 and (W % 32 == 0 or W >= 96):
            form, rows = "wino4", piece(L.CONV3X3_WINO4)
    splits = 1
    if rows and form == "wino4" and k_split and mode in (L.PRO_NONE, L.PRO_AFFINE_SILU):
        splits = int(L.load().nd_conv3x3_wino4_splitk_plan(B, H, W, cin, cout))
    if rows and form == "wino4_16" and k_16split:
        splits = int(L.load().nd_conv3x3_wino4_16_splitk_plan(H, W, cin, cout))
    if splits > 1:
        rows = piece(_FORM_KERNEL[form], splits)
    if rows:
        return form, splits, rows
    for form in ("wino2", "wino") if k_wino2 else ("wino",):
        rows = piece(_FORM_KERNEL[form], mode=stored)
        if rows:
            return form, 1, rows
    return "", 1, B


_LAUNCH_OUT_BYTES = 2 * 1024 ** 3
_FORM_KERNEL = {"": L.CONV3X3_DIRECT, "wino": L.CONV3X3_WINO, "wino2": L.CONV3X3_WINO2, "wino4": L.CONV3X3_WINO4, "wino4_16": L.CONV3X3_WINO4_16}
_MAP_PRODUCERS = ("pos_block1.mlp.1.weight", "pos_block2.mlp.1.weight")


def _blocked_map_rows(C_: int) -> torch.Tensor:
    i = torch.arange(2 * C_)
    c, j = i // 32, i % 32
    return torch.where(j < 16, 16 * c + j, C_ + 16 * c + j - 16)


_CHAIN_SPLIT_LIMIT = (1 << 32) - (1 << 17)


def _split_layer(cin: int, cout: int) -> bool:
    return SPLIT_PW and pointwise_takes(cin, cout, split=True)


def _classify(name: str, shape: Sequence[int]) -> str:
    if ".attn.to_q." in name or ".attn.to_k." in name or ".norm1." in name:
        return "skip"
    if len(shape) == 4:
        k = shape[-1]
        if name == "pos_enc.weights.weight" or name.endswith(".g"):
            return "raw"
        if k == 7:
            return "conv7"
        if k == 3:
            return "conv3"
        if name.startswith("downs.") and name.endswith((".3.1.weight", ".2.1.weight")):
            return "pw_unshuffle"
        return "pw"
    if len(shape) == 2 and (".ff.net." in name):
        return "pw"
    return "raw"


@dataclass
class Slot:
    offset: int
    numel: int
    kind: str
    shape: Tuple[int, ...]


class Engine:

    def __init__(self, dim: int, device: torch.device, mid_attn: bool = False, inp_dim: int = 4, arch: str = "NoiseDiffNet", stage_attn=None):
        if device.type != "cuda":
            raise L.HipError("noisediff_amd runs on MI355X only: got device %r (there is no CPU path)" % (device,))
        self.lib = L.load()
        self.dim, self.device, self.mid_attn, self.inp_dim = dim, device, mid_attn, inp_dim
        self.arch, self.traits = arch, arch_traits(arch)
        self.spec = list(arch_param_spec(arch, dim, inp_dim))
        if mid_attn:
            self.spec += attention_param_spec("mid_attn", 8 * dim)
        self.stage_attn = normalize_stage_attn(stage_attn)
        if self.stage_attn:
            self.spec += stage_attention_param_spec(dim, self.stage_attn)
        self.resnet_names = [p.name[:-len(".mlp.1.weight")] for p in self.spec
                             if p.name.endswith(".mlp.1.weight") and len(p.shape) == 2]
        self.tproj_off: Dict[str, int] = {}
        self._layout()
        with torch.inference_mode(False):
            self.arena = torch.empty(self.arena_floats, dtype=torch.float32, device=device)
        with torch.cuda.device(device):
            s = C.c_void_p()
            L.call("nd_stream_create", C.byref(s))
        self.stream = s
        self.plans: Dict[Tuple[int, int, int], "Plan"] = {}
        self.loaded = False
        self.used: set = set()
        self.valid: Optional[set] = None

    def __del__(self):
        s, self.stream = getattr(self, "stream", None), None
        for q in (s,):
            if q:
                try:
                    L.call("nd_stream_sync", q)
                    L.call("nd_stream_destroy", q)
                except Exception:
                    pass

    def _layout(self) -> None:
        self.slots: Dict[str, Slot] = {}
        off = 0

        def add(name, numel, kind, shape):
            nonlocal off
            self.slots[name] = Slot(off, int(numel), kind, tuple(shape))
            off += (int(numel) + _ALIGN - 1) // _ALIGN * _ALIGN

        for p in self.spec:
            kind = _classify(p.name, p.shape)
            if kind == "skip":
                continue
            if kind == "conv3":
                n = self.lib.nd_pack_conv3x3_weight_floats(p.shape[1], p.shape[0])
                add(p.name + ".wino", self.lib.nd_pack_conv3x3_wino_weight_floats(p.shape[1], p.shape[0]), "derived", p.shape)
                if WINO4 and _wino4_layer(p.shape[1], p.shape[0]):
                    add(p.name + ".wino4", self.lib.nd_pack_conv3x3_wino4_weight_floats(p.shape[1], p.shape[0]), "derived", p.shape)
            elif kind in ("pw", "pw_unshuffle"):
                n = self.lib.nd_pack_pointwise_weight_floats(p.shape[1], p.shape[0])
                if p.name in _MAP_PRODUCERS and p.shape[0] % 32 == 0:
                    add(p.name + ".blk16", n, "derived", p.shape)
                    add(p.name[:-len("weight")] + "bias.blk16", p.shape[0], "derived", (p.shape[0],))
                    if GENMAP and p.shape[1] == POS_DIM == 8 and p.shape[0] % 32 == 0:
                        add(p.name + ".gen", p.shape[0] * p.shape[1], "derived", p.shape)
                if kind == "pw" and p.name.endswith(_CHAIN_FIRST + _CHAIN_LATER):
                    first = int(p.name.endswith(_CHAIN_FIRST))
                    add(p.name + ".chain", self.lib.nd_pack_chain_weight_floats(p.shape[1], p.shape[0], first), "derived", p.shape)
                    if SPLIT_CHAIN:
                        add(p.name + ".chain_s", self.lib.nd_pack_chain_weight_split_floats(p.shape[1], p.shape[0], first), "derived", p.shape)
                if kind == "pw" and _split_layer(p.shape[1], p.shape[0]):
                    add(p.name + ".split", self.lib.nd_pack_pointwise_weight_split_floats(p.shape[1], p.shape[0]), "derived", p.shape)
            elif kind == "conv7":
                n = 196 * p.shape[0]
                if SPLIT_PW and p.name == "init_conv.weight":
                    add(p.name + ".split", self.lib.nd_pack_conv7x7_weight_split_floats(p.shape[0]), "derived", p.shape)
            else:
                n = math.prod(p.shape)
            add(p.name, n, kind, p.shape)
        j = 0
        for r in self.resnet_names:
            self.tproj_off[r] = j
            j += self.slots[r + ".mlp.1.weight"].shape[0]
        self.tproj_rows = j
        add("tproj.weight", j * 4 * self.dim, "derived", (j, 4 * self.dim))
        add("tproj.bias", j, "derived", (j,))
        add("time_freqs", self.dim // 2, "derived", (self.dim // 2,))
        wr, wf = self.slots.get("final_res_block.res_conv.weight"), self.slots.get("final_conv.weight")
        if wr is not None and wf is not None and wf.shape[1] == wr.shape[0] and wr.shape[1] == 2 * wr.shape[0] and \
                self.lib.nd_pointwise_narrow_fold_takes(wr.shape[0], wr.shape[0], wr.shape[0], wf.shape[0]):
            add("final_fold.weight", self.lib.nd_pack_narrow_fold_floats(wr.shape[1] + wr.shape[0], wf.shape[0]), "derived", (wf.shape[0], wr.shape[1] + wr.shape[0]))
            add("final_fold.bias", wf.shape[0], "derived", (wf.shape[0],))
        self.time_table = TIME_TABLE and 4 * self.dim <= 2048 and self.lib.nd_cond_step_lds_bytes(16, self.dim) <= 160 * 1024
        if self.time_table:
            add("time_table", TIME_TABLE_ROWS * 4 * self.dim, "derived", (TIME_TABLE_ROWS, 4 * self.dim))
            if PROJ_TABLE and self.tproj_rows % 4 == 0 and TIME_TABLE_ROWS * self.tproj_rows * 4 <= (192 << 20):
                add("tproj_table", TIME_TABLE_ROWS * self.tproj_rows, "derived", (TIME_TABLE_ROWS, self.tproj_rows))
        self.arena_floats = off

    def view(self, name: str) -> torch.Tensor:
        s = self.slots[name]
        return self.arena[s.offset:s.offset + s.numel]

    def p(self, name: str) -> int:
        s = self.slots[name]
        if self.valid is not None and name not in self.valid:
            raise L.HipError(f"arena slice {name!r} was not part of this rank's weight broadcast (it carried the slices of the plans "
                             "recorded before it): record the plan before Engine.broadcast(only_used=True), or broadcast the whole arena")
        self.used.add(name)
        return self.arena.data_ptr() + 4 * s.offset

    def load_state_dict(self, sd: Dict[str, torch.Tensor]) -> None:
        st = self.stream
        self.valid = None
        keep = []
        used = set(self.used)
        with torch.cuda.device(self.device):
            for p in self.spec:
                if p.name not in self.slots:
                    continue
                t = sd[p.name].detach().to(device=self.device, dtype=torch.float32).contiguous()
                if tuple(t.shape) != tuple(p.shape):
                    raise ValueError(f"{p.name}: shape {tuple(t.shape)} != {tuple(p.shape)}")
                keep.append(t)
                kind = self.slots[p.name].kind
                if kind == "raw":
                    self.view(p.name).copy_(t.reshape(-1))
            torch.cuda.synchronize(self.device)
            for p, t in zip([q for q in self.spec if q.name in self.slots], keep):
                kind, dst = self.slots[p.name].kind, self.p(p.name)
                if kind == "conv3":
                    L.call("nd_pack_conv3x3_weight", t.data_ptr(), dst, p.shape[1], p.shape[0], st)
                    L.call("nd_pack_conv3x3_wino_weight", t.data_ptr(), self.p(p.name + ".wino"), p.shape[1], p.shape[0], st)
                    if p.name + ".wino4" in self.slots:
                        L.call("nd_pack_conv3x3_wino4_weight", t.data_ptr(), self.p(p.name + ".wino4"), p.shape[1], p.shape[0], st)
                elif kind == "pw":
                    L.call("nd_pack_pointwise_weight", t.data_ptr(), dst, p.shape[1], p.shape[0], 0, st)
                    if p.name + ".blk16" in self.slots:
                        perm = _blocked_map_rows(p.shape[0] // 2).to(self.device)
                        tp = t[perm].contiguous()
                        keep.append(tp)
                        L.call("nd_pack_pointwise_weight", tp.data_ptr(), self.p(p.name + ".blk16"), p.shape[1], p.shape[0], 0, st)
                        bname = p.name[:-len("weight")] + "bias"
                        self.view(bname + ".blk16").copy_(sd[bname].detach().to(device=self.device, dtype=torch.float32)[perm])
                    if p.name + ".gen" in self.slots:
                        self.view(p.name + ".gen").copy_(t.reshape(-1))
                    if p.name + ".chain" in self.slots:
                        L.call("nd_pack_chain_weight", t.data_ptr(), self.p(p.name + ".chain"), p.shape[1], p.shape[0],
                               int(p.name.endswith(_CHAIN_FIRST)), st)
                    if p.name + ".chain_s" in self.slots:
                        L.call("nd_pack_chain_weight_split", t.data_ptr(), self.p(p.name + ".chain_s"), p.shape[1], p.shape[0],
                               int(p.name.endswith(_CHAIN_FIRST)), st)
                    if p.name + ".split" in self.slots:
                        L.call("nd_pack_pointwise_weight_split", t.data_ptr(), self.p(p.name + ".split"), p.shape[1], p.shape[0], st)
                elif kind == "pw_unshuffle":
                    L.call("nd_pack_pointwise_weight", t.data_ptr(), dst, p.shape[1], p.shape[0], p.shape[1] // 4, st)
                elif kind == "conv7":
                    L.call("nd_pack_conv7x7_weight", t.data_ptr(), dst, p.shape[0], st)
                    if p.name + ".split" in self.slots:
                        L.call("nd_pack_conv7x7_weight_split", t.data_ptr(), self.p(p.name + ".split"), p.shape[0], st)
            if "final_fold.weight" in self.slots:
                raw = {p.name: t for p, t in zip([q for q in self.spec if q.name in self.slots], keep)}
                wr, wf = raw["final_res_block.res_conv.weight"], raw["final_conv.weight"]
                L.call("nd_pack_narrow_fold", wf.data_ptr(), raw["final_conv.bias"].data_ptr(), wr.data_ptr(), raw["final_res_block.res_conv.bias"].data_ptr(),
                       self.p("final_fold.weight"), self.p("final_fold.bias"), wr.shape[1], wr.shape[0], wf.shape[0], st)
            L.call("nd_stream_sync", st)
            tw = torch.cat([self.view(r + ".mlp.1.weight") for r in self.resnet_names])
            tb = torch.cat([self.view(r + ".mlp.1.bias") for r in self.resnet_names])
            self.view("tproj.weight").copy_(tw)
            self.view("tproj.bias").copy_(tb)
            half = self.dim // 2
            e = math.log(10000) / (half - 1)
            self.view("time_freqs").copy_(torch.exp(torch.arange(half) * -e).to(torch.float32))
            torch.cuda.synchronize(self.device)
            self._build_time_tables()
        self.loaded, self.valid, self.used = True, None, used

    _DERIVED_TABLES = ("time_table", "tproj_table")

    def _build_time_tables(self) -> None:
        if not self.time_table:
            return
        st, used = self.stream, set(self.used)
        with torch.cuda.device(self.device):
            L.call("nd_cond_table_build_f32", self.p("time_freqs"), self.p("time_mlp.1.weight"), self.p("time_mlp.1.bias"), self.p("time_mlp.3.weight"),
                   self.p("time_mlp.3.bias"), self.p("time_table"), TIME_TABLE_ROWS, self.dim, st)
            L.call("nd_stream_sync", st)
            if "tproj_table" in self.slots:
                ts = torch.arange(TIME_TABLE_ROWS, dtype=torch.int64, device=self.device)
                torch.cuda.synchronize(self.device)
                J = self.tproj_rows
                for t0 in range(0, TIME_TABLE_ROWS, 16):
                    nb = min(16, TIME_TABLE_ROWS - t0)
                    L.call("nd_cond_step_table_f32", ts.data_ptr() + 8 * t0, self.p("time_freqs"), self.p("time_mlp.1.weight"), self.p("time_mlp.1.bias"),
                           self.p("time_mlp.3.weight"), self.p("time_mlp.3.bias"), self.p("tproj.weight"), self.p("tproj.bias"),
                           self.p("tproj_table") + 4 * t0 * J, J, nb, self.dim, J, self.p("time_table"), TIME_TABLE_ROWS, st)
                L.call("nd_stream_sync", st)
        self.used = used

    def broadcast_state_dict(self, sd: Optional[Dict[str, torch.Tensor]], src: int = 0, group=None) -> int:
        import torch.distributed as dist
        names = [p for p in self.spec if p.name in self.slots]
        total = sum(math.prod(p.shape) for p in names)
        with torch.cuda.device(self.device), torch.inference_mode(False):
            if dist.get_rank(group) == src:
                flat = torch.cat([sd[p.name].detach().reshape(-1).to(torch.float32) for p in names]).to(self.device)
                if flat.numel() != total:
                    raise ValueError("broadcast_state_dict: the state dict does not match the network's parameter spec")
            else:
                flat = torch.empty(total, dtype=torch.float32, device=self.device)
            torch.cuda.synchronize(self.device)
            dist.broadcast(flat, src=src, group=group)
            torch.cuda.synchronize(self.device)
            views, at = {}, 0
            for p in names:
                n = math.prod(p.shape)
                views[p.name] = flat[at:at + n].view(*p.shape)
                at += n
        self.load_state_dict(views)
        return total * 4

    def broadcast(self, src: int = 0, group=None, only_used: bool = False) -> int:
        import torch.distributed as dist
        with torch.cuda.device(self.device):
            torch.cuda.synchronize(self.device)
            if not only_used:
                dist.broadcast(self.arena, src=src, group=group)
                nbytes = self.arena.numel() * 4
            else:
                tables = [n for n in self._DERIVED_TABLES if n in self.used]
                if tables:
                    for dep in ("time_freqs", "time_mlp.1.weight", "time_mlp.1.bias", "time_mlp.3.weight", "time_mlp.3.bias", "tproj.weight", "tproj.bias"):
                        self.used.add(dep)
                names = sorted((n for n in self.used if n not in self._DERIVED_TABLES), key=lambda n: self.slots[n].offset)
                every = [None] * dist.get_world_size(group)
                dist.all_gather_object(every, names, group=group)
                if any(e != names for e in every):
                    raise L.HipError("Engine.broadcast(only_used=True): the ranks recorded different plans")
                ranges: List[List[int]] = []
                for n in names:
                    sl = self.slots[n]
                    lo, hi = sl.offset, sl.offset + (sl.numel + _ALIGN - 1) // _ALIGN * _ALIGN
                    if ranges and ranges[-1][1] == lo:
                        ranges[-1][1] = hi
                    else:
                        ranges.append([lo, hi])
                is_src = dist.get_rank(group) == src
                with torch.inference_mode(False):
                    stage = (torch.cat([self.arena[lo:hi] for lo, hi in ranges]) if is_src
                             else torch.empty(sum(hi - lo for lo, hi in ranges), dtype=torch.float32, device=self.device))
                dist.broadcast(stage, src=src, group=group)
                if not is_src:
                    at = 0
                    for lo, hi in ranges:
                        self.arena[lo:hi].copy_(stage[at:at + hi - lo])
                        at += hi - lo
                    self.valid = set(names) | set(tables)
                    if tables:
                        torch.cuda.synchronize(self.device)
                        self._build_time_tables()
                nbytes = stage.numel() * 4
            torch.cuda.synchronize(self.device)
        self.loaded = True
        return nbytes

    def copy_from(self, other: "Engine") -> None:
        if other.arena_floats != self.arena_floats or not other.loaded:
            raise L.HipError("Engine.copy_from: the source engine has no weights or another layout")
        other.sync()
        torch.cuda.synchronize(other.device)
        with torch.cuda.device(self.device):
            self.arena.copy_(other.arena)
            torch.cuda.synchronize(self.device)
        self.loaded, self.valid = True, other.valid

    def plan(self, B: int, H: int, W: int, debug: bool = False, tag: int = 0, allow_empty: bool = False) -> "Plan":
        if not self.loaded and not allow_empty:
            raise L.HipError("Engine has no weights: call load_state_dict() or broadcast() first")
        key = (B, H, W, debug, tag)
        if key not in self.plans:
            self.plans[key] = Plan(self, B, H, W, debug)
        return self.plans[key]

    def sync(self) -> None:
        L.call("nd_stream_sync", self.stream)


Op = Tuple[Callable, tuple]


class Plan:

    def __init__(self, eng: Engine, B: int, H: int, W: int, debug: bool = False):
        self.debug, self.taps = debug, {}
        self.lock = threading.Lock()
        if H % 8 or W % 8:
            raise AssertionError(f"your input dimensions {(H, W)} need to be divisible by 8, given the unet")
        self.e, self.B, self.H, self.W = eng, B, H, W
        self.dev = eng.device
        self._keep: List[object] = []
        self._free: Dict[int, List[torch.Tensor]] = {}
        self.workspace_floats = 0
        d = eng.dim
        with torch.cuda.device(self.dev), torch.inference_mode(False):
            f = lambda *s: torch.empty(*s, dtype=torch.float32, device=self.dev)
            self.x = f(B, H, W, eng.inp_dim)
            self.clean = f(B, H, W, eng.inp_dim)
            self.position = f(B, 2, H, W)
            self.iso_idx = torch.zeros(B, dtype=torch.int64, device=self.dev)
            self.time = torch.zeros(B, dtype=torch.int64, device=self.dev)
            self.model_out = f(B, H, W, eng.inp_dim)
            self.nchw_tmp = f(B, eng.inp_dim, H, W)
            self.pos_emb = f(B, H, W, POS_DIM)
            self.posgen = (GENMAP and eng.traits.position and all(b + ".mlp.1.weight.gen" in eng.slots for b in ("pos_block1", "pos_block2")) and d % 16 == 0 and
                           conv3x3_form(B, H, W, d, d, d, 0, d, 0, L.PRO_AFFINE_GENMAP_SILU, False, "pos_block1.block2.proj.weight.wino4" in eng.slots)[0] == "wino4")
            self.posmap1 = self.posmap2 = None
            if self.posgen:
                self.pos_e = f(B, H, W, POS_DIM)
                self.pos_e_mad = torch.tensor([0.0, 1.0, 0.0], device=self.dev).repeat_interleave(POS_DIM).repeat(B).view(B, 3, POS_DIM).contiguous()
            else:
                self.posmap1 = f(B, H, W, 2 * d)
                self.posmap2 = f(B, H, W, 2 * d)
            self.posmap_blocked = (not self.posgen and MAP_BLOCKED and "pos_block1.mlp.1.weight.blk16" in eng.slots and
                                   conv3x3_form(B, H, W, d, d, d, 0, d, 0, L.PRO_AFFINE_MAP_SILU, False, "pos_block1.block2.proj.weight.wino4" in eng.slots)[::2] == ("wino4", B))
            self.iso_emb = f(B, ISO_DIM)
            self.attn_names = [p.name[:-len(".attn.to_v.weight")] for p in eng.spec if p.name.endswith(".attn.to_v.weight")]
            self.cb = {n: f(B, eng.slots[n + ".proj_out.bias"].shape[0]) for n in self.attn_names}
            self.emb = f(B, d)
            self.t1 = f(B, 4 * d)
            self.st = f(B, 4 * d)
            self.tproj = f(B, eng.tproj_rows)
        self.cond_ops: List[Op] = []
        self.step_ops: List[Op] = []
        self._ops = self.cond_ops
        self._record_condition()
        self._ops = self.step_ops
        self._record_time()
        self._record_net()
        self.condition_set = False

    def _alloc(self, *shape) -> torch.Tensor:
        n = math.prod(shape)
        lst = self._free.get(n)
        if lst:
            return lst.pop().view(*shape)
        self.workspace_floats += n
        with torch.cuda.device(self.dev), torch.inference_mode(False):
            t = torch.empty(n, dtype=torch.float32, device=self.dev)
        self._keep.append(t)
        return t.view(*shape)

    def _tap(self, name: str, t: torch.Tensor) -> torch.Tensor:
        if self.debug:
            self.taps[name] = t
        return t

    def _release(self, *ts: torch.Tensor) -> None:
        if self.debug:
            return
        for t in ts:
            self._free.setdefault(t.numel(), []).append(t.reshape(-1))

    def _add(self, name: str, *args, meta: Optional[dict] = None) -> None:
        fn = getattr(self.e.lib, name)
        self._keep.append(args)
        self._ops.append((fn, args, name, meta))

    def _src(self, t: torch.Tensor, t2: Optional[torch.Tensor] = None, mode=L.PRO_NONE, **kw) -> L.Src:
        s = L.Src()
        s.p0, s.c0, s.ld0 = t.data_ptr(), t.shape[-1], t.shape[-1]
        if t2 is not None:
            s.p1, s.c1, s.ld1 = t2.data_ptr(), t2.shape[-1], t2.shape[-1]
        s.mode = mode
        for k, v in kw.items():
            setattr(s, k, v.data_ptr() if isinstance(v, torch.Tensor) else v)
        return s

    def conv3(self, name: str, src: L.Src, cin: int, cout: int, H: int, W: int, stats: bool):
        e = self.e
        out = self._alloc(self.B, H, W, cout)
        up = 1 if src.upsample else 0
        form, splits, rows = conv3x3_form(self.B, H, W, cin, cout, src.c0, src.c1, src.ld0, src.ld1, src.mode, bool(src.upsample), (name + ".weight.wino4") in e.slots)
        wino, wino2, wino4 = form != "", form == "wino2", form.startswith("wino4")
        if src.mode == L.PRO_AFFINE_GENMAP_SILU and form != "wino4":
            raise L.HipError(f"{name}: maps formed in the kernel need conv3x3_wino4's 16 x 32-region form (Plan.posgen decides by the same rule)")
        if wino and not wino4 and (name + ".weight.wino4") in e.slots and src.mode in (L.PRO_NONE, L.PRO_AFFINE_SILU, L.PRO_AFFINE_MAP_SILU) and not _few_items(H, W, cout):
            _log.warning("%s (%d -> %d at %d x %d, batch %d): not on the F(4x4) kernel", name, cin, cout, H, W, self.B)
        st = sc = None
        slots = 0
        if stats:
            slots = (e.lib.nd_conv3x3_wino4_stat_slots(H, W) if wino4 else e.lib.nd_conv3x3_wino_stat_slots(H, W) if wino
                     else e.lib.nd_conv3x3_stat_slots(H, W, cout, self.B))
            st = self._alloc(self.B, slots, cout, 2)
            sc = self._alloc(slots)
        if src.map_blocked and not wino4:
            raise L.HipError(f"{name}: the scale / shift map was produced in the blocked layout but the layer does not run on conv3x3_wino4")
        weight = e.p(name + (".weight.wino4" if wino4 else ".weight.wino" if wino else ".weight"))
        entry = f"nd_conv3x3_{form}_nhwc_f32" if form else "nd_conv3x3_nhwc_f32"
        tiling = (9016 if form == "wino4_16" else 9004) if wino4 else 9002 if wino2 else 9001 if wino else e.lib.nd_conv3x3_tiling_id(self.B, H, W, cout)
        ws = self._alloc(splits * rows * H * W * cout) if splits > 1 else None
        sh, sw, ctot = H >> up, W >> up, src.c0 + src.c1
        for b0 in range(0, self.B, rows):
            nb = min(rows, self.B - b0)
            d = L.Conv3x3()
            s = L.Src.from_buffer_copy(src)
            if b0:
                s.p0 = src.p0 + 4 * b0 * sh * sw * src.ld0
                if src.p1:
                    s.p1 = src.p1 + 4 * b0 * sh * sw * src.ld1
                if src.mad:
                    s.mad = src.mad + 4 * b0 * 3 * ctot
                if src.map:
                    s.map = src.map + 4 * b0 * H * W * (POS_DIM if src.mode == L.PRO_AFFINE_GENMAP_SILU else 2 * ctot)
            d.src, d.weight, d.bias, d.out = s, weight, e.p(name + ".bias"), out.data_ptr() + 4 * b0 * H * W * cout
            d.B, d.H, d.W, d.cin, d.cout, d.ldo = nb, H, W, cin, cout, cout
            if stats:
                d.stats, d.slot_count = st.data_ptr() + 4 * b0 * slots * cout * 2, sc.data_ptr()
            meta = {"layer": name, "B": nb, "H": H, "W": W, "cin": cin, "cout": cout, "mode": int(src.mode), "tiling": tiling}
            if splits > 1:
                meta["splits"] = splits
                self._add(f"nd_conv3x3_{form}_splitk_nhwc_f32", C.byref(d), ws.data_ptr(), splits, e.stream, meta=meta)
            else:
                self._add(entry, C.byref(d), e.stream, meta=meta)
            self._keep.append(d)
        if ws is not None:
            self._release(ws)
        return out, st, sc, slots

    def pw(self, name: str, src: L.Src, cin: int, cout: int, HW: int, W: int, act=L.ACT_NONE, bias=True,
           res0=None, res1=None, vec=None, gn_t=None, gn_mad=None, out=None, variant: str = "") -> torch.Tensor:
        e = self.e
        if out is None:
            out = self._alloc(self.B, HW, cout)
        d = L.Pointwise()
        d.src, d.out = src, out.data_ptr()
        d.bias = e.p(name + ".bias" + variant) if bias else None
        d.B, d.HW, d.W, d.cin, d.cout, d.ldo, d.act = self.B, HW, W, cin, cout, cout, act
        split = not variant and (name + ".weight.split") in e.slots and bool(e.lib.nd_pointwise_gemm_split_takes(C.byref(d)))
        d.weight = e.p(name + (".weight.split" if split else ".weight" + variant))
        if res0 is not None:
            d.res0, d.ldr0 = res0.data_ptr(), res0.shape[-1]
        if res1 is not None:
            d.res1, d.ldr1 = res1.data_ptr(), res1.shape[-1]
        if vec is not None:
            d.vec = vec.data_ptr()
        if gn_t is not None:
            d.gn_t, d.ldt, d.gn_mad = gn_t.data_ptr(), gn_t.shape[-1], gn_mad.data_ptr()
        self._add("nd_pointwise_gemm_split_nhwc_f32" if split else "nd_pointwise_gemm_nhwc_f32", C.byref(d), e.stream,
                  meta={"layer": name, "B": self.B, "HW": HW, "cin": cin, "cout": cout, "split": int(split)})
        self._keep.append(d)
        return out

    def gn_finalize(self, st, sc, slots: int, norm: str, C_: int, groups: int, ss_off: Optional[int]) -> torch.Tensor:
        e = self.e
        mad = self._alloc(self.B, 3, C_)
        ss = (self.tproj.data_ptr() + 4 * ss_off) if ss_off is not None else None
        self._add("nd_groupnorm_finalize_f32", st.data_ptr(), sc.data_ptr(), slots, e.p(norm + ".weight"), e.p(norm + ".bias"),
                  ss, e.tproj_rows, mad.data_ptr(), self.B, C_, groups, GN_EPS, e.stream)
        return mad

    def linear_rows(self, x: torch.Tensor, w: int, b: Optional[int], out: torch.Tensor, K: int, N: int, act_in=0, act_out=0):
        self._add("nd_linear_rows_f32", x.data_ptr(), x.shape[-1], w, b, out.data_ptr(), out.shape[-1], self.B, K, N,
                  act_in, act_out, self.e.stream)

    def resnet(self, name: str, x: torch.Tensor, skip: Optional[torch.Tensor], cout: int, H: int, W: int, groups: int,
               posmap: Optional[torch.Tensor] = None, extra_res: Optional[torch.Tensor] = None, tail: bool = True):
        cin = x.shape[-1] + (skip.shape[-1] if skip is not None else 0)
        HW = H * W
        c1, st1, sc1, n1 = self.conv3(name + ".block1.proj", self._src(x, skip), cin, cout, H, W, stats=True)
        ss_off = None if posmap is not None else self.e.tproj_off.get(name)
        mad1 = self.gn_finalize(st1, sc1, n1, name + ".block1.norm", cout, groups, ss_off)
        a1 = None
        if PREACT and posmap is None and cout >= PREACT_MIN and H >= 16 and W >= 16:
            a1 = self._alloc(self.B, HW, cout)
            self._add("nd_affine_silu_add_f32", c1.data_ptr(), cout, mad1.data_ptr(), None, cout, None, cout, a1.data_ptr(), cout,
                      self.B, HW, cout, self.e.stream,
                      meta={"layer": name + ".block1.act", "stream_bytes": 4.0 * self.B * HW * cout * 2})
            src2 = self._src(a1)
        else:
            if posmap is not None and self.posgen:
                src2 = self._src(c1, None, L.PRO_AFFINE_GENMAP_SILU, mad=mad1, map=self.pos_e, gamma=self.e.p(name + ".mlp.1.weight.gen"),
                                 beta=self.e.p(name + ".mlp.1.bias"))
            else:
                mode = L.PRO_AFFINE_MAP_SILU if posmap is not None else L.PRO_AFFINE_SILU
                src2 = self._src(c1, None, mode, mad=mad1, **({"map": posmap, "map_blocked": int(self.posmap_blocked)} if posmap is not None else {}))
        c2, st2, sc2, n2 = self.conv3(name + ".block2.proj", src2, cout, cout, H, W, stats=True)
        if a1 is not None:
            self._release(a1)
        mad2 = self.gn_finalize(st2, sc2, n2, name + ".block2.norm", cout, groups, None)
        if not tail:
            self._release(c1, st1, sc1, mad1, st2, sc2)
            return c2, mad2
        if cin != cout:
            assert extra_res is None
            out = self.pw(name + ".res_conv", self._src(x, skip), cin, cout, HW, W, gn_t=c2, gn_mad=mad2)
        else:
            assert skip is None
            out = self._alloc(self.B, HW, cout)
            self._add("nd_affine_silu_add_f32", c2.data_ptr(), cout, mad2.data_ptr(), x.data_ptr(), cout,
                      extra_res.data_ptr() if extra_res is not None else None, cout, out.data_ptr(), cout,
                      self.B, HW, cout, self.e.stream,
                      meta={"layer": name + ".tail", "stream_bytes": 4.0 * self.B * HW * cout * (4 if extra_res is not None else 3)})
        self._release(c1, st1, sc1, mad1, c2, st2, sc2, mad2)
        return out.view(self.B, H, W, cout)

    def chain(self, name: str, src: L.Src, stages, HW: int, tail=None) -> torch.Tensor:
        e = self.e
        out = self._alloc(self.B, HW, stages[-1][2])
        split = all((layer + ".weight.chain_s") in e.slots for layer, *_ in stages) and (src.c1 == 0 or stages[0][1] <= 16)
        ldo = stages[-1][2]
        if tail is not None and not split:
            raise L.HipError(f"{name}: the tail prologue is a form of the split chain only")
        rows = self.B
        if split:
            per = 4 * HW * max(src.ld0, src.ld1, ldo, *([t.shape[-1] for t in tail[1:] if t is not None] if tail else []))
            rows = max(1, min(self.B, _CHAIN_SPLIT_LIMIT // per))
            rows = -(-self.B // -(-self.B // rows))
        for b0 in range(0, self.B, rows):
            nb = min(rows, self.B - b0)
            d = L.Chain()
            sp = L.Src.from_buffer_copy(src)
            if b0:
                sp.p0 = src.p0 + 4 * b0 * HW * src.ld0
                if src.p1:
                    sp.p1 = src.p1 + 4 * b0 * HW * src.ld1
                if src.vec:
                    sp.vec = src.vec + 4 * b0 * (src.c0 + src.c1)
            d.src, d.out, d.n_stages, d.B, d.HW, d.ldo = sp, out.data_ptr() + 4 * b0 * HW * ldo, len(stages), nb, HW, ldo
            for i, (layer, cin, cout, act, res) in enumerate(stages):
                d.st[i].weight, d.st[i].bias = e.p(layer + (".weight.chain_s" if split else ".weight.chain")), e.p(layer + ".bias")
                d.st[i].cin, d.st[i].cout, d.st[i].act, d.st[i].res = cin, cout, act, res
            meta = {"layer": name, "B": nb, "HW": HW, "cin": stages[0][1], "cout": stages[-1][2], "split": int(split),
                    "flop_per_px": 2.0 * sum(c_in * c_out for _, c_in, c_out, _, _ in stages)}
            if tail is not None:
                mad, r0, r1 = tail
                dt = L.ChainTail()
                dt.chain, dt.mad = d, mad.data_ptr() + 4 * b0 * 3 * src.c0
                dt.r0, dt.ldr0 = r0.data_ptr() + 4 * b0 * HW * r0.shape[-1], r0.shape[-1]
                if r1 is not None:
                    dt.r1, dt.ldr1 = r1.data_ptr() + 4 * b0 * HW * r1.shape[-1], r1.shape[-1]
                self._add("nd_pointwise_chain_tail_split_nhwc_f32", C.byref(dt), e.stream, meta=meta)
                self._keep.append(dt)
                continue
            self._add("nd_pointwise_chain_split_nhwc_f32" if split else "nd_pointwise_chain_nhwc_f32", C.byref(d), e.stream, meta=meta)
            self._keep.append(d)
        return out

    def _chain_ok(self, HW: int, widths) -> bool:
        return CHAIN and chain_takes(HW, *widths)

    def attn_block(self, name: str, x: torch.Tensor, H: int, W: int) -> torch.Tensor:
        Cc, HW = x.shape[-1], H * W
        cb = self.cb[name]
        if self._chain_ok(HW, (Cc, 2 * Cc, Cc, Cc)):
            ln = self._src(x, None, L.PRO_LAYERNORM, vec=cb, gamma=self.e.p(name + ".norm2.weight"), beta=self.e.p(name + ".norm2.bias"))
            y = self.chain(name + ".ff+proj_out", ln,
                           [(name + ".ff.net.0.0", Cc, 2 * Cc, L.ACT_GELU, L.CHAIN_RES_NONE),
                            (name + ".ff.net.2", 2 * Cc, Cc, L.ACT_NONE, L.CHAIN_RES_INPUT),
                            (name + ".proj_out", Cc, Cc, L.ACT_NONE, L.CHAIN_RES_INPUT_RAW)], HW)
            return y.view(self.B, H, W, Cc)
        kw = {}
        rs = None
        if Cc > 64:
            rs = self._alloc(self.B, HW, 2)
            self._add("nd_layernorm_stats_f32", x.data_ptr(), Cc, cb.data_ptr(), rs.data_ptr(), self.B, HW, Cc, 1e-5, self.e.stream)
            kw["rowstats"] = rs
        ln = self._src(x, None, L.PRO_LAYERNORM, vec=cb, gamma=self.e.p(name + ".norm2.weight"), beta=self.e.p(name + ".norm2.bias"), **kw)
        h1 = self.pw(name + ".ff.net.0.0", ln, Cc, 2 * Cc, HW, W, act=L.ACT_GELU)
        x2 = self.pw(name + ".ff.net.2", self._src(h1), 2 * Cc, Cc, HW, W, res0=x, vec=cb)
        y = self.pw(name + ".proj_out", self._src(x2), Cc, Cc, HW, W, res0=x)
        self._release(h1, x2)
        if rs is not None:
            self._release(rs)
        return y.view(self.B, H, W, Cc)

    def mlp(self, name: str, src: L.Src, cin: int, hid: int, cout: int, H: int, W: int, res0=None) -> torch.Tensor:
        if res0 is None and src.mode == L.PRO_NONE and self._chain_ok(H * W, (cin, hid, cout)):
            o = self.chain(name, src, [(name + ".fc1", cin, hid, L.ACT_GELU, L.CHAIN_RES_NONE),
                                       (name + ".fc2", hid, cout, L.ACT_NONE, L.CHAIN_RES_NONE)], H * W)
            return o.view(self.B, H, W, cout)
        h = self.pw(name + ".fc1", src, cin, hid, H * W, W, act=L.ACT_GELU)
        o = self.pw(name + ".fc2", self._src(h), hid, cout, H * W, W, res0=res0)
        self._release(h)
        return o.view(self.B, H, W, cout)

    def _record_condition(self) -> None:
        e, B, H, W, st = self.e, self.B, self.H, self.W, self.e.stream
        tr = e.traits
        if tr.position:
            pe = self._alloc(B, H, W, 3 * POS_DIM)
            self._add("nd_pos_enc_f32", self.position.data_ptr(), e.p("pos_enc.weights.weight"), e.p("pos_enc.weights.bias"),
                      pe.data_ptr(), B, H, W, POS_DIM, st)
            h = self.pw("pos_mlp.fc1", self._src(pe), 3 * POS_DIM, 2 * POS_DIM, H * W, W, act=L.ACT_GELU)
            self.pw("pos_mlp.fc2", self._src(h), 2 * POS_DIM, POS_DIM, H * W, W, out=self.pos_emb)
            if self.posgen:
                self._add("nd_affine_silu_add_f32", self.pos_emb.data_ptr(), POS_DIM, self.pos_e_mad.data_ptr(), None, POS_DIM, None, POS_DIM,
                          self.pos_e.data_ptr(), POS_DIM, B, H * W, POS_DIM, st, meta={"layer": "pos_emb.silu", "stream_bytes": 8.0 * B * H * W * POS_DIM})
            for blk, dst in (() if self.posgen else (("pos_block1", self.posmap1), ("pos_block2", self.posmap2))):
                self.pw(blk + ".mlp.1", self._src(self.pos_emb, None, L.PRO_SILU), POS_DIM, 2 * e.dim, H * W, W, out=dst,
                        variant=".blk16" if self.posmap_blocked else "")
            self._release(pe, h)
        if tr.iso_attn:
            self._add("nd_embedding_rows_f32", self.iso_idx.data_ptr(), e.p("iso_embed.weight"), self.iso_emb.data_ptr(), B,
                      ISO_TABLE_ROWS, ISO_DIM, st)
            inner = ATTN_HEADS * ATTN_DIM_HEAD
            v = self._alloc(B, inner)
            for n in self.attn_names:
                Cc = self.cb[n].shape[-1]
                self.linear_rows(self.iso_emb, e.p(n + ".attn.to_v.weight"), None, v, ISO_DIM, inner)
                self.linear_rows(v, e.p(n + ".attn.to_out.0.weight"), e.p(n + ".attn.to_out.0.bias"), self.cb[n], inner, Cc)
            self._release(v)
        self.clean_emb = None
        if tr.cond_branch:
            ce = self._alloc(B, H, W, e.dim)
            self._add("nd_conv7x7_c4_f32", self.clean.data_ptr(), e.p("cond_init_conv.weight"), e.p("cond_init_conv.bias"),
                      ce.data_ptr(), e.dim, B, H, W, e.dim, st)
            self.clean_emb = self._tap("clean_emb", self.resnet("cond_res_block1", ce, None, e.dim, H, W, RESNET_GROUPS))
            self._release(ce)

    def _record_time(self) -> None:
        e, d = self.e, self.e.dim
        if COND_STEP and 4 * d <= 2048 and e.lib.nd_cond_step_lds_bytes(self.B, d) <= 160 * 1024:
            args = (self.time.data_ptr(), e.p("time_freqs"), e.p("time_mlp.1.weight"), e.p("time_mlp.1.bias"),
                    e.p("time_mlp.3.weight"), e.p("time_mlp.3.bias"), e.p("tproj.weight"), e.p("tproj.bias"), self.tproj.data_ptr(),
                    e.tproj_rows, self.B, d, e.tproj_rows)
            if e.time_table and "tproj_table" in e.slots and e.tproj_rows % 4 == 0:
                self._add("nd_cond_step_ptable_f32", *args, e.p("time_table"), TIME_TABLE_ROWS, e.p("tproj_table"), e.stream)
            elif e.time_table:
                self._add("nd_cond_step_table_f32", *args, e.p("time_table"), TIME_TABLE_ROWS, e.stream)
            else:
                self._add("nd_cond_step_f32", *args, e.stream)
            return
        self._add("nd_sinusoidal_time_emb_f32", self.time.data_ptr(), e.p("time_freqs"), self.emb.data_ptr(), self.B, d // 2, e.stream)
        self.linear_rows(self.emb, e.p("time_mlp.1.weight"), e.p("time_mlp.1.bias"), self.t1, d, 4 * d, act_out=L.ACT_GELU)
        self.linear_rows(self.t1, e.p("time_mlp.3.weight"), e.p("time_mlp.3.bias"), self.st, 4 * d, 4 * d, act_out=L.ACT_SILU)
        self.linear_rows(self.st, e.p("tproj.weight"), e.p("tproj.bias"), self.tproj, 4 * d, e.tproj_rows)

    def _record_net(self) -> None:
        e, B, H, W, d = self.e, self.B, self.H, self.W, self.e.dim
        G, tr = RESNET_GROUPS, self.e.traits
        shot_noise = None
        if tr.shot_branch:
            r_shot = self.mlp("shot_mlp1", self._src(self.clean, self.x), 2 * e.inp_dim, d, d, H, W)
            s = self.attn_block("shot_attn", r_shot, H, W)
            s2 = self.mlp("shot_mlp2", self._src(s), d, d, d, H, W)
            if (SHOT_TAIL and not self.debug and SPLIT_CHAIN and self._chain_ok(H * W, (d, d, e.inp_dim)) and e.lib.nd_pointwise_chain_tail_takes(d, d, e.inp_dim, 0)
                    and all(n + ".weight.chain_s" in e.slots for n in ("shot_mlp3.fc1", "shot_mlp3.fc2"))):
                c2, mad2 = self.resnet("shot_time", s2, None, d, H, W, SHOT_GROUPS, tail=False)
                shot_noise = self.chain("shot_time.tail+shot_mlp3", self._src(c2), [("shot_mlp3.fc1", d, d, L.ACT_GELU, L.CHAIN_RES_NONE),
                                                                                   ("shot_mlp3.fc2", d, e.inp_dim, L.ACT_NONE, L.CHAIN_RES_NONE)], H * W,
                                        tail=(mad2, s2, r_shot)).view(B, H, W, e.inp_dim)
                self._release(r_shot, s, s2, c2, mad2)
                s3 = None
            else:
                s3 = self.resnet("shot_time", s2, None, d, H, W, SHOT_GROUPS, extra_res=r_shot)
                shot_noise = self._tap("shot_noise", self.mlp("shot_mlp3", self._src(s3), d, d, e.inp_dim, H, W))
            if s3 is not None:
                for nm, tt in (("shot_mlp1", r_shot), ("shot_attn", s), ("shot_mlp2", s2), ("shot_time", s3)):
                    self._tap(nm, tt)
                self._release(r_shot, s, s2, s3)
        x0 = self._alloc(B, H, W, d)
        stem_split = "init_conv.weight.split" in e.slots
        self._add("nd_conv7x7_c4_split_f32" if stem_split else "nd_conv7x7_c4_f32", self.x.data_ptr(),
                  e.p("init_conv.weight.split" if stem_split else "init_conv.weight"), e.p("init_conv.bias"), x0.data_ptr(), d, B, H, W, d, e.stream)
        self._tap("init_conv", x0)
        xin = x0
        if tr.cond_branch:
            xin, *_ = self.conv3("cond_concat_conv", self._src(x0, self.clean_emb), 2 * d, d, H, W, stats=False)
            self._tap("cond_concat", xin)
        pm1, pm2 = ((self.pos_e, self.pos_e) if self.posgen else (self.posmap1, self.posmap2)) if tr.position else (None, None)
        x = self._tap("pos_block1", self.resnet("pos_block1", xin, None, d, H, W, POS_GROUPS, posmap=pm1))
        if xin is not x0:
            self._release(xin)
        rs = 3 if tr.iso_attn else 2
        hs: List[torch.Tensor] = []
        h, w = H, W
        for i, (cin, cout) in enumerate(stage_dims(d)):
            p = f"downs.{i}"
            x1 = self.resnet(p + ".0", x, None, cin, h, w, G)
            self._release(x)
            x2 = self.resnet(p + ".1", x1, None, cin, h, w, G)
            if e.stage_attn and e.stage_attn[i]:
                x2 = self._stage_attention(f"down_attns.{i}", e.stage_attn[i], x2, h, w)
            hs += [x1, x2]
            xa = self.attn_block(p + ".2", x2, h, w) if tr.iso_attn else x2
            self._tap(p + ".0", x1); self._tap(p + ".1", x2); self._tap(p + ".2", xa)
            if i == 3:
                x, *_ = self.conv3(f"{p}.{rs}", self._src(xa), cin, cout, h, w, stats=False)
            else:
                h, w = h // 2, w // 2
                x = self.pw(f"{p}.{rs}.1", self._src(xa, None, L.PRO_NONE, unshuffle=1, c0=4 * cin, ld0=cin), 4 * cin, cout,
                            h * w, w).view(B, h, w, cout)
            if xa is not x2:
                self._release(xa)
            self._tap(f"down{i}", x)
        mid = x.shape[-1]
        xm = self.resnet("mid_block1", x, None, mid, h, w, G)
        self._release(x)
        if e.mid_attn:
            xm = self._mid_attention(xm, h, w)
        x = self._tap("mid", self.resnet("mid_block2", xm, None, mid, h, w, G))
        self._release(xm)
        for i, (cin, cout) in enumerate(reversed(stage_dims(d))):
            p = f"ups.{i}"
            sk = hs.pop()
            x1 = self.resnet(p + ".0", x, sk, cout, h, w, G)
            self._release(x, sk)
            sk = hs.pop()
            x2 = self.resnet(p + ".1", x1, sk, cout, h, w, G)
            self._release(x1, sk)
            if e.stage_attn and e.stage_attn[3 - i]:
                x2 = self._stage_attention(f"up_attns.{i}", e.stage_attn[3 - i], x2, h, w)
            xa = self.attn_block(p + ".2", x2, h, w) if tr.iso_attn else x2
            if xa is not x2:
                self._release(x2)
            if i == 3:
                x, *_ = self.conv3(f"{p}.{rs}", self._src(xa), cout, cin, h, w, stats=False)
            else:
                h, w = h * 2, w * 2
                x, *_ = self.conv3(f"{p}.{rs}.1", self._src(xa, None, L.PRO_NONE, upsample=1), cout, cin, h, w, stats=False)
            self._release(xa)
            self._tap(p + ".0", x1); self._tap(p + ".1", x2); self._tap(p + ".2", xa); self._tap(f"up{i}", x)
        xp = self._tap("pos_block2", self.resnet("pos_block2", x, None, d, H, W, POS_GROUPS, posmap=pm2))
        self._release(x)
        if FOLD_FINAL and not self.debug and "final_fold.weight" in e.slots:
            c2, mad2 = self.resnet("final_res_block", xp, x0, d, H, W, G, tail=False)
            nf = L.NarrowFold()
            nf.p0, nf.p1, nf.t, nf.mad = xp.data_ptr(), x0.data_ptr(), c2.data_ptr(), mad2.data_ptr()
            nf.weight, nf.bias, nf.out = e.p("final_fold.weight"), e.p("final_fold.bias"), self.model_out.data_ptr()
            nf.B, nf.HW, nf.c0, nf.c1, nf.c2, nf.ld0, nf.ld1, nf.ldt, nf.cout, nf.ldo = B, H * W, d, d, d, d, d, d, e.inp_dim, e.inp_dim
            if shot_noise is not None:
                nf.res0, nf.ldr0 = shot_noise.data_ptr(), e.inp_dim
            self._add("nd_pointwise_narrow_fold_nhwc_f32", C.byref(nf), e.stream,
                      meta={"layer": "final_res_block.res_conv+final_conv", "B": B, "HW": H * W, "cin": 3 * d, "cout": e.inp_dim})
            self._keep.append(nf)
            self._release(xp, x0, c2, mad2)
            if shot_noise is not None:
                self._release(shot_noise)
            return
        xf = self._tap("final_res_block", self.resnet("final_res_block", xp, x0, d, H, W, G))
        self._release(xp, x0)
        self.pw("final_conv", self._src(xf), d, e.inp_dim, H * W, W, res0=shot_noise, out=self.model_out)
        self._release(xf)
        if shot_noise is not None:
            self._release(shot_noise)

    def _mid_attention(self, x: torch.Tensor, h: int, w: int, prefix: str = "mid_attn") -> torch.Tensor:
        e, B, Cc, N = self.e, self.B, x.shape[-1], h * w
        hid = ATTN_HEADS * ATTN_DIM_HEAD
        xn = self._alloc(B, N, Cc)
        self._add("nd_rmsnorm_nhwc_f32", x.data_ptr(), Cc, e.p(prefix + ".norm.g"), xn.data_ptr(), Cc, B, N, Cc, e.stream)
        qkv = self.pw(prefix + ".to_qkv", self._src(xn), Cc, 3 * hid, N, w, bias=False)
        att = self._alloc(B, N, hid)
        self._add("nd_attention_mfma_f32", qkv.data_ptr(), 3 * hid, att.data_ptr(), hid, B, N, ATTN_HEADS, ATTN_DIM_HEAD, e.stream)
        y = self.pw(prefix + ".to_out", self._src(att), hid, Cc, N, w, res0=x)
        self._release(xn, qkv, att, x)
        return y.view(B, h, w, Cc)

    def _stage_attention(self, prefix: str, kind: str, x: torch.Tensor, h: int, w: int) -> torch.Tensor:
        if kind == "full":
            return self._mid_attention(x, h, w, prefix)
        e, B, Cc, N = self.e, self.B, x.shape[-1], h * w
        hid = ATTN_HEADS * ATTN_DIM_HEAD
        xn = self._alloc(B, N, Cc)
        self._add("nd_rmsnorm_nhwc_f32", x.data_ptr(), Cc, e.p(prefix + ".norm.g"), xn.data_ptr(), Cc, B, N, Cc, e.stream)
        qkv = self.pw(prefix + ".to_qkv", self._src(xn), Cc, 3 * hid, N, w, bias=False)
        att = self._alloc(B, N, hid)
        ws = self._alloc(int(e.lib.nd_linear_attention_workspace_floats(B, N, ATTN_HEADS)))
        self._add("nd_linear_attention_f32", qkv.data_ptr(), 3 * hid, att.data_ptr(), hid, ws.data_ptr(), B, N, ATTN_HEADS, ATTN_DIM_HEAD, e.stream)
        o = self.pw(prefix + ".to_out.0", self._src(att), hid, Cc, N, w)
        y = self._alloc(B, N, Cc)
        self._add("nd_rmsnorm_add_nhwc_f32", o.data_ptr(), Cc, e.p(prefix + ".to_out.1.g"), x.data_ptr(), Cc, y.data_ptr(), Cc, B, N, Cc, e.stream)
        self._release(xn, qkv, att, ws, o, x)
        return y.view(B, h, w, Cc)

    @staticmethod
    def run(ops: List[Op]) -> None:
        for fn, args, name, _meta in ops:
            r = fn(*args)
            if r != 0:
                L.check(r, name)

    def set_condition(self, condition) -> None:
        B, H, W, e = self.B, self.H, self.W, self.e
        tr = e.traits
        if torch.is_tensor(condition):
            if tr.position or tr.iso_attn:
                raise TypeError(f"{e.arch} needs the condition dict (clean_img, position, iso_ratio_idx), got a tensor")
            condition = {"clean_img": condition}
        clean = condition["clean_img"]
        if tuple(clean.shape) != (B, e.inp_dim, H, W):
            raise ValueError(f"condition shapes: clean_img {tuple(clean.shape)} do not match batch {(B, e.inp_dim, H, W)}")
        with torch.cuda.device(self.dev):
            self.nchw_tmp.copy_(clean.to(self.dev, torch.float32))
            if tr.position:
                pos = condition["position"]
                if tuple(pos.shape) != (B, 2, H, W):
                    raise ValueError(f"condition shapes: position {tuple(pos.shape)} do not match batch {(B, 2, H, W)}")
                self.position.copy_(pos.to(self.dev, torch.float32))
            if tr.iso_attn:
                iso = condition["iso_ratio_idx"]
                if tuple(iso.shape) != (B,):
                    raise ValueError(f"condition shapes: iso_ratio_idx {tuple(iso.shape)} do not match batch {(B,)}")
                iso = iso.to(torch.int64)
                if int(iso.min()) < 0 or int(iso.max()) >= ISO_TABLE_ROWS:
                    raise IndexError("iso_ratio_idx out of range for nn.Embedding(100, 16)")
                self.iso_idx.copy_(iso.to(self.dev))
            torch.cuda.synchronize(self.dev)
            L.call("nd_nchw_to_nhwc_f32", self.nchw_tmp.data_ptr(), self.clean.data_ptr(), B, e.inp_dim, H, W, e.stream)
            self.run(self.cond_ops)
            e.sync()
        self.condition_set = True

    def load_x(self, x_nchw: torch.Tensor) -> None:
        e = self.e
        with torch.cuda.device(self.dev):
            self.nchw_tmp.copy_(x_nchw.to(self.dev, torch.float32))
            torch.cuda.synchronize(self.dev)
            L.call("nd_nchw_to_nhwc_f32", self.nchw_tmp.data_ptr(), self.x.data_ptr(), self.B, e.inp_dim, self.H, self.W, e.stream)

    def read_nchw(self, nhwc: torch.Tensor) -> torch.Tensor:
        e = self.e
        with torch.cuda.device(self.dev), torch.inference_mode(False):
            out = torch.empty(self.B, e.inp_dim, self.H, self.W, dtype=torch.float32, device=self.dev)
            L.call("nd_nhwc_to_nchw_f32", nhwc.data_ptr(), out.data_ptr(), self.B, e.inp_dim, self.H, self.W, e.stream)
            e.sync()
        return out

    def forward(self, x_nchw: torch.Tensor, time: torch.Tensor) -> torch.Tensor:
        if not self.condition_set:
            raise L.HipError("Plan.forward: set_condition() first")
        with torch.cuda.device(self.dev):
            self.time.copy_(time.to(self.dev, torch.int64))
        self.load_x(x_nchw)
        self.run(self.step_ops)
        return self.read_nchw(self.model_out)
```

Baseline: 0.9543 patches/s.

## Fuse resnet tail affine+SiLU+residual into LayerNorm attention FF chain

Adds a three-stage LayerNorm form of the pointwise chain tail kernel. It applies the second resnet block's GroupNorm affine, SiLU and residual as a prologue, writes the intermediate x2 out for the skip connection, then runs the FF and proj_out GEMMs in the same kernel. This removes a separate kernel launch and a full read and write round trip of x2 at the high-resolution down stage. Row prefetches are also moved into the middle of the GEMM loops to overlap loads with compute. The cost is a larger template instantiation with more register pressure and a new code path that only applies to cin=64 at HW of at least 128x128.

```diff
diff --git a/include/noisediff_hip.h b/include/noisediff_hip.h
--- a/include/noisediff_hip.h
+++ b/include/noisediff_hip.h
@@ -307,9 +307,13 @@
     const float* r0;
     const float* r1;
     int32_t  ldr0, ldr1;
+    float*   y;
+    int32_t  ldy, reserved;
 } nd_chain_tail;
 int nd_pointwise_chain_tail_split_nhwc_f32(const nd_chain_tail* d, void* stream);
 int nd_pointwise_chain_tail_takes(int cin, int n1, int n2, int n3);
+int nd_pointwise_chain_tail_ln_supported(int cin, int n1, int n2, int n3);
+int nd_pointwise_chain_tail_ln_takes(int HW, int cin, int n1, int n2, int n3);
 
 
 int nd_groupnorm_finalize_f32(const float* stats, const float* slot_count, int slots,
diff --git a/noisediff_amd/_lib.py b/noisediff_amd/_lib.py
--- a/noisediff_amd/_lib.py
+++ b/noisediff_amd/_lib.py
@@ -61,7 +61,8 @@
 
 
 class ChainTail(C.Structure):
-    _fields_ = [("chain", Chain), ("mad", fptr), ("r0", fptr), ("r1", fptr), ("ldr0", C.c_int32), ("ldr1", C.c_int32)]
+    _fields_ = [("chain", Chain), ("mad", fptr), ("r0", fptr), ("r1", fptr), ("ldr0", C.c_int32), ("ldr1", C.c_int32),
+                ("y", fptr), ("ldy", C.c_int32), ("reserved", C.c_int32)]
 
 
 class NarrowFold(C.Structure):
@@ -168,6 +169,8 @@
     "nd_pack_pointwise_weight_split": (i32, [vp, vp, i32, i32, vp]),
     "nd_pointwise_chain_tail_split_nhwc_f32": (i32, [C.POINTER(ChainTail), vp]),
     "nd_pointwise_chain_tail_takes": (i32, [i32, i32, i32, i32]),
+    "nd_pointwise_chain_tail_ln_supported": (i32, [i32, i32, i32, i32]),
+    "nd_pointwise_chain_tail_ln_takes": (i32, [i32, i32, i32, i32, i32]),
     "nd_pointwise_narrow_fold_nhwc_f32": (i32, [C.POINTER(NarrowFold), vp]),
     "nd_pointwise_narrow_fold_takes": (i32, [i32, i32, i32, i32]),
     "nd_pack_narrow_fold_floats": (i64, [i32, i32]),
@@ -289,7 +292,7 @@
 
 _UNCHECKED = {"nd_conv3x3_takes", "nd_pointwise_gemm_takes", "nd_pointwise_gemm_split_takes", "nd_pointwise_chain_supported", "nd_pointwise_chain_takes",
               "nd_groupnorm_train_takes", "nd_layernorm_train_takes", "nd_rmsnorm_train_takes", "nd_token_sum_takes", "nd_conv3x3_wgrad_plan", "nd_conv3x3_wgrad_cat_takes",
-              "nd_pointwise_chain_tail_takes", "nd_pointwise_narrow_fold_takes", "nd_pack_narrow_fold_floats", "nd_version", "nd_last_error", "nd_stream_device", "nd_conv3x3_wgrad_form", "nd_adam_chunk_elements", "nd_ema_chunk_elements", "nd_conv7x7_c4_wgrad_workspace_floats", "nd_conv3x3_stat_slots", "nd_conv3x3_tiling_id", "nd_pack_conv3x3_weight_floats",
+              "nd_pointwise_chain_tail_takes", "nd_pointwise_chain_tail_ln_supported", "nd_pointwise_chain_tail_ln_takes", "nd_pointwise_narrow_fold_takes", "nd_pack_narrow_fold_floats", "nd_version", "nd_last_error", "nd_stream_device", "nd_conv3x3_wgrad_form", "nd_adam_chunk_elements", "nd_ema_chunk_elements", "nd_conv7x7_c4_wgrad_workspace_floats", "nd_conv3x3_stat_slots", "nd_conv3x3_tiling_id", "nd_pack_conv3x3_weight_floats",
               "nd_pack_pointwise_weight_floats", "nd_linear_attention_workspace_floats", "nd_conv3x3_wino_stat_slots", "nd_conv3x3_wino4_stat_slots",
               "nd_pack_conv3x3_wino_weight_floats", "nd_pack_conv3x3_wino4_weight_floats", "nd_conv3x3_wino4_splitk_plan", "nd_conv3x3_wino4_16_splitk_plan", "nd_conv3x3_wino4_splitk_workspace_floats", "nd_token_sum_workspace_floats", "nd_cond_step_lds_bytes", "nd_conv3x3_wgrad_workspace_floats",
               "nd_groupnorm_train_workspace_floats", "nd_linear_wgrad_workspace_floats",
diff --git a/noisediff_amd/csrc/pwchain.hip b/noisediff_amd/csrc/pwchain.hip
--- a/noisediff_amd/csrc/pwchain.hip
+++ b/noisediff_amd/csrc/pwchain.hip
@@ -12,6 +12,8 @@
     const float* r0;
     const float* r1;
     int ldr0, ldr1;
+    float* y;
+    int ldy;
 };
 
 template <int K, int N>
@@ -36,9 +38,10 @@
         }
 }
 
-template <int K, int N>
+struct chain_no_mid { __device__ __forceinline__ void operator()() const {} };
+template <int K, int N, class Mid = chain_no_mid>
 __device__ __forceinline__ void chain_gemm_split(const float (&in)[K / 2], const char* __restrict__ w, const float* __restrict__ bias,
-                                                 f32x16 (&acc)[N / 32], const int lane) {
+                                                 f32x16 (&acc)[N / 32], const int lane, const Mid& mid = Mid()) {
     static_assert(K % 16 == 0, "whole 16-channel K steps");
     constexpr int S = K / 16, NT = N / 32;
     const int half = lane >> 5;
@@ -71,6 +74,7 @@
 #pragma unroll
         for (int nt = 0; nt < NT; ++nt) {
             const int g = s * NT + nt;
+            if (s == S / 2 && nt == 0) mid();
             if (g + 1 < S * NT) load_w((g + 1) & 1, nt + 1 < NT ? s : s + 1, nt + 1 < NT ? nt + 1 : 0);
             __builtin_amdgcn_sched_barrier(0);
             if (nt == 0 && s + 1 < S) split((s + 1) & 1, s + 1);
@@ -117,6 +121,11 @@
         }
 }
 
+__device__ __forceinline__ f32x4 chain_add_rounded(const f32x4 a, const f32x4 b) {
+#pragma clang fp contract(off)
+    return a + b;
+}
+
 template <int N>
 __device__ __forceinline__ void chain_store_buf(const f32x16 (&acc)[N / 32], __amdgpu_buffer_rsrc_t rso, const unsigned row_bytes, const int cout, const int half) {
 #pragma unroll
@@ -156,11 +165,13 @@
 
 template <bool SPLIT> constexpr int chain_w_floats(int n, int k) { return SPLIT ? n * k * 3 / 2 : n * k; }
 
-template <int K0, int N1, int N2, int N3, int MODE, bool SPLIT = false, bool TAIL = false>
+template <int K0, int N1, int N2, int N3, int MODE, bool SPLIT = false, bool TAIL = false, bool R1 = TAIL>
 __global__ __launch_bounds__(chain_threads(N1, SPLIT, K0), 1) void chain_kernel(const ChainArgs a) {
     constexpr int THREADS = chain_threads(N1, SPLIT, K0), WAVES = THREADS / 64;
+    constexpr bool THROUGH = TAIL && MODE == ND_PRO_LAYERNORM;
     static_assert(!SPLIT || K0 % 16 == 0, "SPLIT: the first stage reads whole 16-channel K steps");
-    static_assert(!TAIL || (SPLIT && MODE == ND_PRO_NONE), "TAIL: a prologue of the SPLIT form");
+    static_assert(!TAIL || (SPLIT && (MODE == ND_PRO_NONE || MODE == ND_PRO_LAYERNORM)), "TAIL: a prologue of the SPLIT form");
+    static_assert(TAIL || !R1, "R1: the tail's second residual");
     extern __shared__ __attribute__((aligned(16))) float lds[];
     float* w1 = lds;
     float* w2 = w1 + chain_w_floats<SPLIT>(N1, K0);
@@ -175,7 +186,7 @@
 
     const int tid = threadIdx.x, lane = tid & 63, wave = tid >> 6, half = lane >> 5;
     const nd_src& s = a.d.src;
-    const int cin = s.c0 + s.c1;
+    const int cin = s.c0 + s.c1, c0 = THROUGH ? K0 : s.c0, ca = THROUGH ? K0 : cin;
 
     {
         auto copy4 = [&](float* dst, const float* src, int n) {
@@ -204,7 +215,7 @@
     float* myv = vst + wave * K0;
     float* mym = mst + wave * 3 * K0;
     int b_cur = -1;
-    const int cout_last = a.d.st[N3 > 0 ? 2 : 1].cout;
+    const int cout_last = THROUGH ? N3 : a.d.st[N3 > 0 ? 2 : 1].cout;
 
     constexpr bool TWO = SPLIT && K0 == 16;
     constexpr unsigned OOB = 0xFFFFFFF0u;
@@ -216,24 +227,31 @@
                                                                           TAIL ? (int)((unsigned)a.d.B * a.d.HW * a.ldr0 * 4u) : 0, 0x00020000);
     const __amdgpu_buffer_rsrc_t rr1 = __builtin_amdgcn_make_buffer_rsrc(const_cast<float*>(TAIL && a.r1 ? a.r1 : s.p0), 0,
                                                                           TAIL && a.r1 ? (int)((unsigned)a.d.B * a.d.HW * a.ldr1 * 4u) : 0, 0x00020000);
+    const __amdgpu_buffer_rsrc_t rsy = __builtin_amdgcn_make_buffer_rsrc(THROUGH && a.y ? a.y : const_cast<float*>(s.p0), 0,
+                                                                          THROUGH && a.y ? (int)((unsigned)a.d.B * a.d.HW * a.ldy * 4u) : 0, 0x00020000);
     f32x4 Xn[SPLIT ? K0 / 8 : 1], Xm[TWO ? K0 / 8 : 1];
-    f32x4 R0n[TAIL ? K0 / 8 : 1], R1n[TAIL ? K0 / 8 : 1];
-    auto prefetch_rows = [&](int t_) {
+    f32x4 R0n[TAIL ? K0 / 8 : 1], R1n[R1 ? K0 / 8 : 1];
+    auto prefetch_rows = [&](int t_, auto rows, auto res) {
         const unsigned pix_ = (unsigned)t_ * 32u + (unsigned)(lane & 31);
 #pragma unroll
         for (int q = 0; q < K0 / 8; ++q) {
             const int c = 8 * q + 4 * half;
-            Xn[SPLIT ? q : 0] = __builtin_bit_cast(f32x4, __builtin_amdgcn_raw_buffer_load_b128(rs0, c < s.c0 ? (pix_ * (unsigned)s.ld0 + c) * 4u : OOB, 0, 0));
-            if constexpr (TWO)
-                Xm[q] = __builtin_bit_cast(f32x4, __builtin_amdgcn_raw_buffer_load_b128(rs1, (c >= s.c0 && c < cin) ? (pix_ * (unsigned)s.ld1 + (c - s.c0)) * 4u : OOB, 0, 0));
-            if constexpr (TAIL) {
-                R0n[q] = __builtin_bit_cast(f32x4, __builtin_amdgcn_raw_buffer_load_b128(rr0, c < cin ? (pix_ * (unsigned)a.ldr0 + c) * 4u : OOB, 0, 0));
-                R1n[q] = __builtin_bit_cast(f32x4, __builtin_amdgcn_raw_buffer_load_b128(rr1, c < cin ? (pix_ * (unsigned)a.ldr1 + c) * 4u : OOB, 0, 0));
+            if constexpr (rows.value) {
+                Xn[SPLIT ? q : 0] = __builtin_bit_cast(f32x4, __builtin_amdgcn_raw_buffer_load_b128(rs0, c < c0 ? (pix_ * (unsigned)s.ld0 + c) * 4u : OOB, 0, 0));
+                if constexpr (TWO)
+                    Xm[q] = __builtin_bit_cast(f32x4, __builtin_amdgcn_raw_buffer_load_b128(rs1, (c >= s.c0 && c < cin) ? (pix_ * (unsigned)s.ld1 + (c - s.c0)) * 4u : OOB, 0, 0));
+            }
+            if constexpr (TAIL && res.value) {
+                R0n[q] = __builtin_bit_cast(f32x4, __builtin_amdgcn_raw_buffer_load_b128(rr0, c < ca ? (pix_ * (unsigned)a.ldr0 + c) * 4u : OOB, 0, 0));
+                if constexpr (R1)
+                    R1n[q] = __builtin_bit_cast(f32x4, __builtin_amdgcn_raw_buffer_load_b128(rr1, c < cin ? (pix_ * (unsigned)a.ldr1 + c) * 4u : OOB, 0, 0));
             }
         }
     };
+    constexpr std::true_type yes{};
+    constexpr std::false_type no{};
     if constexpr (SPLIT) {
-        if (t_begin < t_end) prefetch_rows(t_begin);
+        if (t_begin < t_end) prefetch_rows(t_begin, yes, yes);
     }
 
 #ifdef CHAIN_STAMP
@@ -244,14 +262,15 @@
         CH_T0();
         const int b = t / a.tiles_per_sample;
         const size_t pix = (size_t)t * 32 + (lane & 31);
-        if (s.vec && b != b_cur) {
-            for (int c = lane; c < K0; c += 64) myv[c] = c < cin ? s.vec[(size_t)b * cin + c] : 0.0f;
-            b_cur = b;
-        }
-        if (TAIL && b != b_cur) {
-            for (int c = lane; c < 3 * K0; c += 64) {
-                const int j = c / K0, cc = c - j * K0;
-                mym[c] = cc < cin ? a.mad[((size_t)b * 3 + j) * cin + cc] : 0.0f;
+        if (b != b_cur) {
+            if (s.vec) {
+                for (int c = lane; c < K0; c += 64) myv[c] = c < cin ? s.vec[(size_t)b * cin + c] : 0.0f;
+            }
+            if (TAIL) {
+                for (int c = lane; c < 3 * K0; c += 64) {
+                    const int j = c / K0, cc = c - j * K0;
+                    mym[c] = cc < cin ? a.mad[((size_t)b * 3 + j) * cin + cc] : 0.0f;
+                }
             }
             b_cur = b;
         }
@@ -263,10 +282,18 @@
                 if constexpr (TWO) X[q] += Xm[q];
                 if constexpr (TAIL) {
                     const float* m = mym + 8 * q + 4 * half;
-                    X[q] = nd_silu4((X[q] - nd_ld4(m)) * nd_ld4(m + K0) + nd_ld4(m + 2 * K0)) + R0n[q] + R1n[q];
+                    if constexpr (R1) X[q] = nd_silu4((X[q] - nd_ld4(m)) * nd_ld4(m + K0) + nd_ld4(m + 2 * K0)) + R0n[q] + R1n[q];
+                    else X[q] = chain_add_rounded(nd_silu4((X[q] - nd_ld4(m)) * nd_ld4(m + K0) + nd_ld4(m + 2 * K0)), R0n[q]);
                 }
             }
-            prefetch_rows(t + 1 < t_end ? t + 1 : t);
+            if constexpr (THROUGH) {
+#pragma unroll
+                for (int q = 0; q < K0 / 8; ++q) {
+                    const int c = 8 * q + 4 * half;
+                    __builtin_amdgcn_raw_buffer_store_b128(__builtin_bit_cast(u32x4, X[q]), rsy, c < ca ? ((unsigned)pix * (unsigned)a.ldy + c) * 4u : OOB, 0, 0);
+                }
+            } else
+                prefetch_rows(t + 1 < t_end ? t + 1 : t, yes, yes);
             if (s.vec) {
 #pragma unroll
                 for (int q = 0; q < K0 / 8; ++q) X[q] += nd_ld4(myv + 8 * q + 4 * half);
@@ -314,7 +341,9 @@
 
         CH_ACC(0);
         f32x16 H1[N1 / 32];
-        if constexpr (SPLIT) chain_gemm_split<K0, N1>(in0, reinterpret_cast<const char*>(w1), b1, H1, lane);
+        if constexpr (THROUGH)
+            chain_gemm_split<K0, N1>(in0, reinterpret_cast<const char*>(w1), b1, H1, lane, [&] { prefetch_rows(t + 1 < t_end ? t + 1 : t, yes, no); });
+        else if constexpr (SPLIT) chain_gemm_split<K0, N1>(in0, reinterpret_cast<const char*>(w1), b1, H1, lane);
         else chain_gemm<K0, N1>(in0, w1, b1, H1, lane);
         CH_ACC(1);
         chain_res<K0, N1>(H1, X, s.vec ? myv : nullptr, a.d.st[0].res, half);
@@ -326,7 +355,9 @@
 #pragma unroll
             for (int r = 0; r < 16; ++r) in1[16 * nt + r] = H1[nt][r];
         f32x16 H2[N2 / 32];
-        if constexpr (SPLIT) chain_gemm_split<N1, N2>(in1, reinterpret_cast<const char*>(w2), b2, H2, lane);
+        if constexpr (THROUGH)
+            chain_gemm_split<N1, N2>(in1, reinterpret_cast<const char*>(w2), b2, H2, lane, [&] { prefetch_rows(t + 1 < t_end ? t + 1 : t, no, yes); });
+        else if constexpr (SPLIT) chain_gemm_split<N1, N2>(in1, reinterpret_cast<const char*>(w2), b2, H2, lane);
         else chain_gemm<N1, N2>(in1, w2, b2, H2, lane);
         CH_ACC(3);
         chain_res<K0, N2>(H2, X, s.vec ? myv : nullptr, a.d.st[1].res, half);
@@ -387,17 +418,17 @@
     }
 }
 
-template <int K0, int N1, int N2, int N3, int MODE, bool SPLIT = false, bool TAIL = false>
+template <int K0, int N1, int N2, int N3, int MODE, bool SPLIT = false, bool TAIL = false, bool R1 = TAIL>
 int launch(const ChainArgs& a, hipStream_t st) {
     static nd_device_once configured;
     constexpr int THREADS = chain_threads(N1, SPLIT, K0), WAVES = THREADS / 64;
     constexpr int STASH = (TAIL ? 4 : 1) * K0;
     const size_t lds = (size_t)(chain_w_floats<SPLIT>(N1, K0) + chain_w_floats<SPLIT>(N2, N1) + chain_w_floats<SPLIT>(N3, N2) + N1 + N2 + N3 + 2 * K0 + WAVES * STASH) * sizeof(float);
     static_assert((size_t)(chain_w_floats<SPLIT>(N1, K0) + chain_w_floats<SPLIT>(N2, N1) + chain_w_floats<SPLIT>(N3, N2) + N1 + N2 + N3 + 2 * K0 + 16 * STASH) * 4 <= 160 * 1024, "LDS");
-    if (int e = nd_reserve_lds(configured, reinterpret_cast<const void*>(chain_kernel<K0, N1, N2, N3, MODE, SPLIT, TAIL>), lds, "nd_pointwise_chain")) return e;
+    if (int e = nd_reserve_lds(configured, reinterpret_cast<const void*>(chain_kernel<K0, N1, N2, N3, MODE, SPLIT, TAIL, R1>), lds, "nd_pointwise_chain")) return e;
     const int wgs = nd_cdiv(a.n_tiles, WAVES);
     const int grid = wgs < nd_device_cus() ? wgs : nd_device_cus();
-    hipLaunchKernelGGL((chain_kernel<K0, N1, N2, N3, MODE, SPLIT, TAIL>), dim3(grid), dim3(THREADS), lds, st, a);
+    hipLaunchKernelGGL((chain_kernel<K0, N1, N2, N3, MODE, SPLIT, TAIL, R1>), dim3(grid), dim3(THREADS), lds, st, a);
     return 0;
 }
 
@@ -511,40 +542,61 @@
     return n3 == 0 && (cin == 64 || cin == 48) && nd_round_up(n1, 32) == 64 && n1 > 0 && nd_round_up(n2, 32) == 32 && n2 > 0;
 }
 
+extern "C" int nd_pointwise_chain_tail_ln_supported(int cin, int n1, int n2, int n3) {
+    return cin == 64 && n1 > 0 && nd_round_up(n1, 32) == 128 && n2 > 0 && nd_round_up(n2, 32) == 64 && n3 == 64;
+}
+
+extern "C" int nd_pointwise_chain_tail_ln_takes(int HW, int cin, int n1, int n2, int n3) {
+    return chain_pixels_ok(HW) && HW >= 128 * 128 && nd_pointwise_chain_tail_ln_supported(cin, n1, n2, n3);
+}
+
 extern "C" int nd_pointwise_chain_tail_split_nhwc_f32(const nd_chain_tail* dt, void* stream) {
     ND_REQUIRE(dt, ND_E_BADARG, "nd_pointwise_chain_tail: null descriptor");
     const nd_chain* d = &dt->chain;
     const nd_src& s = d->src;
-    ND_REQUIRE(d->n_stages == 2 && s.p0 && d->out && dt->mad && dt->r0, ND_E_BADARG, "nd_pointwise_chain_tail: two stages, t, mad, r0 and out");
+    ND_REQUIRE((d->n_stages == 2 || d->n_stages == 3) && s.p0 && d->out && dt->mad && dt->r0, ND_E_BADARG, "nd_pointwise_chain_tail: two or three stages, t, mad, r0 and out");
+    const bool ln = d->n_stages == 3;
     ND_REQUIRE(d->B > 0 && chain_pixels_ok(d->HW), ND_E_SHAPE, "nd_pointwise_chain_tail: HW=%d must be a positive multiple of 32", d->HW);
-    ND_REQUIRE(s.c1 == 0 && !s.p1 && s.mode == ND_PRO_NONE && !s.vec && !s.upsample && !s.unshuffle && !s.rowstats, ND_E_BADARG,
+    ND_REQUIRE(s.c1 == 0 && !s.p1 && !s.upsample && !s.unshuffle && !s.rowstats, ND_E_BADARG,
                "nd_pointwise_chain_tail: one plain source (the affine + SiLU is this entry point's own prologue)");
+    if (ln) {
+        ND_REQUIRE(s.mode == ND_PRO_LAYERNORM && s.gamma && s.beta && !dt->r1, ND_E_BADARG,
+                   "nd_pointwise_chain_tail: three stages run behind LayerNorm (gamma, beta) of the row with one residual");
+    } else {
+        ND_REQUIRE(s.mode == ND_PRO_NONE && !s.vec && !dt->y, ND_E_BADARG,
+                   "nd_pointwise_chain_tail: one plain source (the affine + SiLU is this entry point's own prologue); vec and y are the three-stage form's");
+    }
     const int cin = s.c0;
-    ND_REQUIRE(nd_pointwise_chain_tail_takes(cin, d->st[0].cout, d->st[1].cout, 0), ND_E_SHAPE,
-               "nd_pointwise_chain_tail: widths %d->%d->%d are not instantiated (nd_affine_silu_add_f32, then the chain)", cin, d->st[0].cout, d->st[1].cout);
-    ND_REQUIRE(s.ld0 >= cin && s.ld0 % 4 == 0 && dt->ldr0 >= cin && dt->ldr0 % 4 == 0 && (!dt->r1 || (dt->ldr1 >= cin && dt->ldr1 % 4 == 0)), ND_E_ALIGN,
-               "nd_pointwise_chain_tail: pixel strides must be >= channels and multiples of 4");
+    ND_REQUIRE(ln ? nd_pointwise_chain_tail_ln_supported(cin, d->st[0].cout, d->st[1].cout, d->st[2].cout) : nd_pointwise_chain_tail_takes(cin, d->st[0].cout, d->st[1].cout, 0), ND_E_SHAPE,
+               "nd_pointwise_chain_tail: widths %d->%d->%d->%d are not instantiated (nd_affine_silu_add_f32, then the chain)", cin, d->st[0].cout, d->st[1].cout,
+               ln ? d->st[2].cout : 0);
+    ND_REQUIRE(s.ld0 >= cin && s.ld0 % 4 == 0 && dt->ldr0 >= cin && dt->ldr0 % 4 == 0 && (!dt->r1 || (dt->ldr1 >= cin && dt->ldr1 % 4 == 0)) &&
+               (!dt->y || (dt->ldy >= cin && dt->ldy % 4 == 0)), ND_E_ALIGN, "nd_pointwise_chain_tail: pixel strides must be >= channels and multiples of 4");
     int width = cin;
-    for (int i = 0; i < 2; ++i) {
+    for (int i = 0; i < d->n_stages; ++i) {
         const nd_chain_stage& g = d->st[i];
-        ND_REQUIRE(g.weight && g.cin == width && g.cout > 0 && g.res == ND_CHAIN_RES_NONE, ND_E_SHAPE, "nd_pointwise_chain_tail: stage %d is %d->%d, expected input width %d, no residual",
-                   i, g.cin, g.cout, width);
+        ND_REQUIRE(g.weight && g.cin == width && g.cout > 0 && (ln ? (g.res == ND_CHAIN_RES_NONE || g.cout == cin) : g.res == ND_CHAIN_RES_NONE), ND_E_SHAPE,
+                   "nd_pointwise_chain_tail: stage %d is %d->%d, expected input width %d, %s", i, g.cin, g.cout, width,
+                   ln ? "a residual needs cout == input width" : "no residual");
         ND_REQUIRE(nd_aligned16(g.weight), ND_E_ALIGN, "nd_pointwise_chain_tail: weights must be 16-byte aligned");
         width = g.cout;
     }
     ND_REQUIRE(width % 4 == 0 && d->ldo >= width && d->ldo % 4 == 0, ND_E_SHAPE, "nd_pointwise_chain_tail: output width %d, ldo %d", width, d->ldo);
-    ND_REQUIRE(nd_aligned16(s.p0) && nd_aligned16(d->out) && nd_aligned16(dt->mad) && nd_aligned16(dt->r0) && nd_aligned16(dt->r1), ND_E_ALIGN,
+    ND_REQUIRE(nd_aligned16(s.p0) && nd_aligned16(d->out) && nd_aligned16(dt->mad) && nd_aligned16(dt->r0) && nd_aligned16(dt->r1) && nd_aligned16(dt->y), ND_E_ALIGN,
                "nd_pointwise_chain_tail: tensors must be 16-byte aligned");
     const long px = (long)d->B * d->HW, lim = (1L << 32) - 65536;
-    ND_REQUIRE(px * s.ld0 * 4 < lim && px * dt->ldr0 * 4 < lim && px * (dt->r1 ? dt->ldr1 : 0) * 4 < lim && px * d->ldo * 4 < lim, ND_E_SHAPE,
-               "nd_pointwise_chain_tail: a tensor of 4 GiB or more");
+    ND_REQUIRE(px * s.ld0 * 4 < lim && px * dt->ldr0 * 4 < lim && px * (dt->r1 ? dt->ldr1 : 0) * 4 < lim && px * d->ldo * 4 < lim &&
+               px * (dt->y ? dt->ldy : 0) * 4 < lim, ND_E_SHAPE, "nd_pointwise_chain_tail: a tensor of 4 GiB or more");
     ChainArgs a{};
     a.d = *d;
     a.tiles_per_sample = d->HW / 32;
     ND_REQUIRE(px / 32 < (1L << 31), ND_E_SHAPE, "nd_pointwise_chain_tail: too many pixels");
     a.n_tiles = (int)(px / 32);
     a.mad = dt->mad;  a.r0 = dt->r0;  a.r1 = dt->r1;  a.ldr0 = dt->ldr0;  a.ldr1 = dt->r1 ? dt->ldr1 : 0;
-    const int rc = cin == 64 ? launch<64, 64, 32, 0, ND_PRO_NONE, true, true>(a, (hipStream_t)stream) : launch<48, 64, 32, 0, ND_PRO_NONE, true, true>(a, (hipStream_t)stream);
+    a.y = dt->y;  a.ldy = dt->y ? dt->ldy : 0;
+    hipStream_t st = (hipStream_t)stream;
+    const int rc = ln ? launch<64, 128, 64, 64, ND_PRO_LAYERNORM, true, true, false>(a, st)
+                      : cin == 64 ? launch<64, 64, 32, 0, ND_PRO_NONE, true, true>(a, st) : launch<48, 64, 32, 0, ND_PRO_NONE, true, true>(a, st);
     if (rc) return rc;
     return nd_launch_status("nd_pointwise_chain_tail_split_nhwc_f32");
 }
diff --git a/noisediff_amd/engine.py b/noisediff_amd/engine.py
--- a/noisediff_amd/engine.py
+++ b/noisediff_amd/engine.py
@@ -38,6 +38,7 @@
 SPLIT_CHAIN, SPLIT_PW = _SPLIT in ("1", "chain"), _SPLIT in ("1", "pw")
 FOLD_FINAL = os.environ.get("ND_FOLD_FINAL", "1") != "0"
 SHOT_TAIL = os.environ.get("ND_SHOT_TAIL", "1") != "0"
+ATTN_TAIL = os.environ.get("ND_ATTN_TAIL", "1") != "0"
 TIME_TABLE = True
 PROJ_TABLE = True
 TIME_TABLE_ROWS = 1000
@@ -645,7 +646,7 @@
         self._release(c1, st1, sc1, mad1, c2, st2, sc2, mad2)
         return out.view(self.B, H, W, cout)
 
-    def chain(self, name: str, src: L.Src, stages, HW: int, tail=None) -> torch.Tensor:
+    def chain(self, name: str, src: L.Src, stages, HW: int, tail=None, y: Optional[torch.Tensor] = None) -> torch.Tensor:
         e = self.e
         out = self._alloc(self.B, HW, stages[-1][2])
         split = all((layer + ".weight.chain_s") in e.slots for layer, *_ in stages) and (src.c1 == 0 or stages[0][1] <= 16)
@@ -654,7 +655,7 @@
             raise L.HipError(f"{name}: the tail prologue is a form of the split chain only")
         rows = self.B
         if split:
-            per = 4 * HW * max(src.ld0, src.ld1, ldo, *([t.shape[-1] for t in tail[1:] if t is not None] if tail else []))
+            per = 4 * HW * max(src.ld0, src.ld1, ldo, *([t.shape[-1] for t in tail[1:] + (y,) if t is not None] if tail else []))
             rows = max(1, min(self.B, _CHAIN_SPLIT_LIMIT // per))
             rows = -(-self.B // -(-self.B // rows))
         for b0 in range(0, self.B, rows):
@@ -680,6 +681,8 @@
                 dt.r0, dt.ldr0 = r0.data_ptr() + 4 * b0 * HW * r0.shape[-1], r0.shape[-1]
                 if r1 is not None:
                     dt.r1, dt.ldr1 = r1.data_ptr() + 4 * b0 * HW * r1.shape[-1], r1.shape[-1]
+                if y is not None:
+                    dt.y, dt.ldy = y.data_ptr() + 4 * b0 * HW * y.shape[-1], y.shape[-1]
                 self._add("nd_pointwise_chain_tail_split_nhwc_f32", C.byref(dt), e.stream, meta=meta)
                 self._keep.append(dt)
                 continue
@@ -690,15 +693,27 @@
     def _chain_ok(self, HW: int, widths) -> bool:
         return CHAIN and chain_takes(HW, *widths)
 
-    def attn_block(self, name: str, x: torch.Tensor, H: int, W: int) -> torch.Tensor:
+    def _attn_stages(self, name: str, Cc: int):
+        return [(name + ".ff.net.0.0", Cc, 2 * Cc, L.ACT_GELU, L.CHAIN_RES_NONE),
+                (name + ".ff.net.2", 2 * Cc, Cc, L.ACT_NONE, L.CHAIN_RES_INPUT),
+                (name + ".proj_out", Cc, Cc, L.ACT_NONE, L.CHAIN_RES_INPUT_RAW)]
+
+    def _attn_tail_ok(self, name: str, Cc: int, HW: int) -> bool:
+        return bool(ATTN_TAIL and not self.debug and SPLIT_CHAIN and self._chain_ok(HW, (Cc, 2 * Cc, Cc, Cc))
+                    and self.e.lib.nd_pointwise_chain_tail_ln_takes(HW, Cc, 2 * Cc, Cc, Cc)
+                    and all(layer + ".weight.chain_s" in self.e.slots for layer, *_ in self._attn_stages(name, Cc)))
+
+    def attn_block(self, name: str, x: torch.Tensor, H: int, W: int, tail=None) -> torch.Tensor:
         Cc, HW = x.shape[-1], H * W
         cb = self.cb[name]
+        if tail is not None:
+            c2, mad2, r0 = tail
+            ln = self._src(c2, None, L.PRO_LAYERNORM, vec=cb, gamma=self.e.p(name + ".norm2.weight"), beta=self.e.p(name + ".norm2.bias"))
+            y = self.chain(name + ".tail+ff+proj_out", ln, self._attn_stages(name, Cc), HW, tail=(mad2, r0, None), y=x)
+            return y.view(self.B, H, W, Cc)
         if self._chain_ok(HW, (Cc, 2 * Cc, Cc, Cc)):
             ln = self._src(x, None, L.PRO_LAYERNORM, vec=cb, gamma=self.e.p(name + ".norm2.weight"), beta=self.e.p(name + ".norm2.bias"))
-            y = self.chain(name + ".ff+proj_out", ln,
-                           [(name + ".ff.net.0.0", Cc, 2 * Cc, L.ACT_GELU, L.CHAIN_RES_NONE),
-                            (name + ".ff.net.2", 2 * Cc, Cc, L.ACT_NONE, L.CHAIN_RES_INPUT),
-                            (name + ".proj_out", Cc, Cc, L.ACT_NONE, L.CHAIN_RES_INPUT_RAW)], HW)
+            y = self.chain(name + ".ff+proj_out", ln, self._attn_stages(name, Cc), HW)
             return y.view(self.B, H, W, Cc)
         kw = {}
         rs = None
@@ -820,11 +835,18 @@
             p = f"downs.{i}"
             x1 = self.resnet(p + ".0", x, None, cin, h, w, G)
             self._release(x)
-            x2 = self.resnet(p + ".1", x1, None, cin, h, w, G)
-            if e.stage_attn and e.stage_attn[i]:
-                x2 = self._stage_attention(f"down_attns.{i}", e.stage_attn[i], x2, h, w)
-            hs += [x1, x2]
-            xa = self.attn_block(p + ".2", x2, h, w) if tr.iso_attn else x2
+            if tr.iso_attn and not (e.stage_attn and e.stage_attn[i]) and x1.shape[-1] == cin and self._attn_tail_ok(p + ".2", cin, h * w):
+                c2, mad2 = self.resnet(p + ".1", x1, None, cin, h, w, G, tail=False)
+                x2 = self._alloc(B, h * w, cin).view(B, h, w, cin)
+                xa = self.attn_block(p + ".2", x2, h, w, tail=(c2, mad2, x1))
+                self._release(c2, mad2)
+                hs += [x1, x2]
+            else:
+                x2 = self.resnet(p + ".1", x1, None, cin, h, w, G)
+                if e.stage_attn and e.stage_attn[i]:
+                    x2 = self._stage_attention(f"down_attns.{i}", e.stage_attn[i], x2, h, w)
+                hs += [x1, x2]
+                xa = self.attn_block(p + ".2", x2, h, w) if tr.iso_attn else x2
             self._tap(p + ".0", x1); self._tap(p + ".1", x2); self._tap(p + ".2", xa)
             if i == 3:
                 x, *_ = self.conv3(f"{p}.{rs}", self._src(xa), cin, cout, h, w, stats=False)
```

Result: no change. 0.9588 patches/s, median of 3 (+0.5%).
